# google-research/frame-interpolation

Hardware: NVIDIA H100
Metric: interpolated_frames_per_sec_1080p (higher is better)
Workload: dtype f16x2-split (activations/weights as fp16 hi+lo planes; fp32 accumulate)

## Files before the change

frame_interpolation_b200/csrc/film_conv.h:

```cpp
#pragma once
#include <cuda.h>
#include <stdint.h>

#include "film_common.cuh"

namespace film {

constexpr int kMaxSrc = 4;
constexpr int kMaxTaps = 9;
constexpr int kChunk = 64;
constexpr int kTileM = 128;

struct ConvSrc {
  const sp_t* hi;
  const sp_t* lo;
  int C;
  int c_off;
  int nchunk;
  int bswap;
};

struct alignas(64) ConvProblem {
  CUtensorMap tm_a_hi[kMaxSrc];
  CUtensorMap tm_a_lo[kMaxSrc];
  CUtensorMap tm_w_hi;
  CUtensorMap tm_w_lo;
  CUtensorMap tm_w_hi_half;
  CUtensorMap tm_w_lo_half;
  ConvSrc src[kMaxSrc];
  int nsrc;
  int B, H, W;
  int tile_h, tile_w;
  int tiles_y, tiles_x;
  int ntaps;
  int tap_dy[kMaxTaps], tap_dx[kMaxTaps];
  int kchunk;
  int ktot;
  const sp_t* w_hi;
  const sp_t* w_lo;
  const float* bias;
  int cout;
  int act;
  sp_t* out_hi;
  sp_t* out_lo;
  int out_C, out_c_off;
  int out_H, out_W;
  int out_sy, out_sx, out_oy, out_ox;
  int epi_mode;
  const float* head_w3;
  const float* head_b3;
  int crop_y, crop_x, crop_h, crop_w;
  int64_t crop_pitch;
  const float* head_w4;
  const float* head_b4;
  const float* head_vup;
  float* head_res;
  float* head_v;
  int v2_resident;
  int v2_na, v2_nw;
  int v2_grid;
  int v2_part_lo, v2_part_hi;
  sp_t* pool_hi;
  sp_t* pool_lo;
  int pool_C;
  int group;
  int pair;
  int halo;
  int bn;
  int passes;
  int straight;
  int out_lo_skip;
};

cudaError_t launch_conv_tc(const ConvProblem* d_prob, const ConvProblem& h_prob, cudaStream_t st);
cudaError_t launch_conv_simt(const ConvProblem* d_prob, const ConvProblem& h_prob, cudaStream_t st);
cudaError_t conv_tc_configure();
bool conv3x3_tc_plan(ConvProblem& h_prob, int num_sms);
void conv3x3_tc_pick_tile(int H, int W, int B, int cout, int kc, int passes, int ktot, int epi_mode, int num_sms,
                          int& tile_h, int& tile_w);
cudaError_t launch_conv3x3_tc(const ConvProblem* d_prob, const ConvProblem& h_prob, cudaStream_t st);
cudaError_t conv3x3_tc_configure();
}
```

frame_interpolation_b200/csrc/film_conv3x3_tc.cu:

```cuda
#include <cuda.h>
#include <cuda_runtime.h>
#include <stdint.h>

#include <type_traits>

#include "film_conv.h"
#include "film_tc_ptx.cuh"

namespace film {
namespace {
using namespace tc;

constexpr int kConsumers = 256;
constexpr int kThreads = kConsumers + 128;
__host__ __device__ constexpr int a_plane_bytes(int kc, int th, int tw) { return (th + 2) * tw * kc * 2; }
__host__ __device__ constexpr int a_stage_bytes(int kc, int th, int tw) { return 2 * a_plane_bytes(kc, th, tw); }
constexpr int kHaloW = 10, kHaloRows = 18;
__host__ __device__ constexpr int halo_box_bytes(int kc) { return kHaloRows * kHaloW * kc * 2; }
__host__ __device__ constexpr int halo_plane_bytes(int kc) { return (halo_box_bytes(kc) + 1023) & ~1023; }
__host__ __device__ constexpr int a_stage_bytes_h(int kc, int th, int tw, int halo, int planes = 2) {
  return planes * (halo ? halo_plane_bytes(kc) : a_plane_bytes(kc, th, tw));
}
constexpr int kMaxRing = 8;
constexpr int kSmemLimit = 227 * 1024;
constexpr int kBarBytes = 8 * (4 * kMaxRing + 4);
constexpr int kFixedBytes = kBarBytes + 16 + 512 * 4  + 64  + 1024  + 64;
constexpr int kHeadW3 = 64 * 32 * 4, kHeadMisc = 512;
constexpr int kHeadBytes = kHeadW3 + kHeadMisc;

__host__ __device__ inline int w_tap_bytes(int bn, int kc, int planes = 2) { return bn * kc * 2 * planes; }

template <int BN, int KC, bool kPartial, bool kHalo, bool kOne, bool kRes>
__global__ void __launch_bounds__(kThreads, 1) k_conv3x3_tc(const ConvProblem* __restrict__ prob) {
  extern __shared__ uint8_t smem_raw[];
  constexpr bool one = kOne;
  const int planes = one ? 1 : 2;
  constexpr int kWPlane = BN * KC * 2;
  const int kWTap = kWPlane * planes;
  const int kTileH = prob->tile_h, kTileW = prob->tile_w;
  constexpr int kHaloBox = halo_box_bytes(KC), kHaloPlane = halo_plane_bytes(KC);
  constexpr bool halo = kHalo;
  const int kAPlane = halo ? kHaloPlane : a_plane_bytes(KC, kTileH, kTileW);
  const int kAStage = planes * kAPlane;
  const int kRowStep = kTileW * KC * 2;
  constexpr bool kFused = BN <= 128;
  constexpr int kAccRegs = (kFused ? 2 * BN : BN) / 2;

  const int NA = prob->v2_na, NW = prob->v2_nw;
  const bool resident = prob->v2_resident != 0;
  const int nsrc = prob->nsrc;
  const int tiles_x = prob->tiles_x, tiles_per_img = prob->tiles_y * prob->tiles_x;
  const int cout = prob->cout;
  const int n_nt = (cout + BN - 1) / BN;
  const int ntiles = prob->B * tiles_per_img * n_nt;
  int nkb = 0;
  for (int s = 0; s < nsrc; ++s) nkb += prob->src[s].nchunk * 9;

  const FastDiv div_nt(n_nt, ntiles), div_img(tiles_per_img, ntiles), div_tx(tiles_x, ntiles);
  const bool pair = prob->pair != 0;
  const int rank = pair ? (int)cluster_ctarank() : 0;
  const int nsp = prob->B * tiles_per_img;
  const int nwork = pair ? ((nsp + 1) / 2) * n_nt : ntiles;
  const int w_first = pair ? (int)blockIdx.x >> 1 : (int)blockIdx.x, w_step = pair ? (int)gridDim.x >> 1 : (int)gridDim.x;
  auto decode = [&](int work, int& sp, int& nti) {
    div_nt.divmod(work, sp, nti);
    if (pair) sp = 2 * sp + rank;
  };

  const uint32_t raw = smem_u32(smem_raw);
  const uint32_t base = (raw + 1023u) & ~1023u;
  uint8_t* gen_base = smem_raw + (base - raw);
  const uint32_t a_base = base;
  const uint32_t w_base = a_base + (uint32_t)NA * kAStage;
  const uint32_t w_bytes = resident ? (uint32_t)nkb * kWTap : (uint32_t)NW * kWTap;
  const uint32_t tail = w_base + w_bytes;
  const uint32_t tail_off = (uint32_t)NA * kAStage + w_bytes;
  float* bias_smem = reinterpret_cast<float*>(gen_base + tail_off + kBarBytes + 16);
  int* src_tab = reinterpret_cast<int*>(gen_base + tail_off + kBarBytes + 16 + 512 * 4);

  const int warp = threadIdx.x >> 5, lane = threadIdx.x & 31;

  if (warp == 8 && lane == 0) {
    for (int s = 0; s < kMaxRing; ++s) {
      mbar_init(tail + 8u * s, 1);
      mbar_init(tail + 8u * (kMaxRing + s), 2);
      mbar_init(tail + 8u * (2 * kMaxRing + s), 1);
      mbar_init(tail + 8u * (3 * kMaxRing + s), pair ? 4 : 2);
    }
    for (int s = 0; s < kMaxSrc; ++s) {
      src_tab[2 * s] = s < nsrc ? prob->src[s].nchunk : 0;
      src_tab[2 * s + 1] = s < nsrc ? prob->src[s].c_off : 0;
      src_tab[2 * kMaxSrc + s] = s < nsrc ? prob->src[s].bswap : 0;
    }
    asm volatile("fence.mbarrier_init.release.cluster;" ::: "memory");
  }
  if (warp < 8)
    for (int i = threadIdx.x; i < n_nt * BN; i += kConsumers) bias_smem[i] = (i < cout) ? prob->bias[i] : 0.f;
  __syncthreads();
  if (pair) cluster_sync_all();
  auto leave = [&]() {
    if (pair) cluster_sync_all();
  };

  if (warp >= 8) {
    regs_dec<40>();
    if (warp > 8) {
      leave();
      return;
    }
    const CUtensorMap* tm_w_hi = &prob->tm_w_hi;
    const CUtensorMap* tm_w_lo = &prob->tm_w_lo;
    if (resident && elect_one()) {
      mbar_expect_tx(tail + 8u * (2 * kMaxRing), (uint32_t)nkb * kWTap);
      for (int kb = 0; kb < nkb; ++kb) {
        tma_load_2d(w_base + kb * kWTap, tm_w_hi, tail + 8u * (2 * kMaxRing), kb * KC, 0);
        if (!one) tma_load_2d(w_base + kb * kWTap + kWPlane, tm_w_lo, tail + 8u * (2 * kMaxRing), kb * KC, 0);
      }
    }
    __syncwarp();
    RingPos ra, rw;
    for (int tile = w_first; tile < nwork; tile += w_step) {
      int sp, nti, b, rem, ty, tx;
      decode(tile, sp, nti);
      div_img.divmod(sp, b, rem);
      div_tx.divmod(rem, ty, tx);
      const int n0 = nti * BN, y0 = ty * kTileH, x0 = tx * kTileW;
      {
        const int nt = tile + w_step;
        int next_sp, nnt;
        decode(nt < nwork ? nt : 0, next_sp, nnt);
        if (nt < nwork && next_sp != sp && next_sp < nsp && elect_one()) {
          int nb, nrem, nty, ntx;
          div_img.divmod(next_sp, nb, nrem);
          div_tx.divmod(nrem, nty, ntx);
          const int ny0 = nty * kTileH, nx0 = ntx * kTileW;
          for (int s = 0; s < nsrc; ++s)
            for (int ch = 0; ch < src_tab[2 * s]; ++ch) {
              const int cc = src_tab[2 * s + 1] + ch * KC;
              tma_prefetch_4d(&prob->tm_a_hi[s], cc, nx0 - 1, ny0 - 1, nb);
              if (!one) tma_prefetch_4d(&prob->tm_a_lo[s], cc, nx0 - 1, ny0 - 1, nb);
              if (!halo) {
                tma_prefetch_4d(&prob->tm_a_hi[s], cc, nx0 + 1, ny0 - 1, nb);
                if (!one) tma_prefetch_4d(&prob->tm_a_lo[s], cc, nx0 + 1, ny0 - 1, nb);
              }
            }
        }
        __syncwarp();
      }
      int kb = 0;
      for (int s = 0; s < nsrc; ++s) {
        const int nchunk = src_tab[2 * s], c_off = src_tab[2 * s + 1];
        const int bs = src_tab[2 * kMaxSrc + s] ? prob->B - 1 - b : b;
        const CUtensorMap* tm_hi = &prob->tm_a_hi[s];
        const CUtensorMap* tm_lo = &prob->tm_a_lo[s];
        for (int ch = 0; ch < nchunk; ++ch) {
          const int nst = halo ? 1 : 3;
          for (int dx = 0; dx < nst; ++dx) {
            const int st = ra.stage;
            mbar_wait(tail + 8u * (kMaxRing + st), ra.phase ^ 1u);
            if (elect_one()) {
              const uint32_t sa = a_base + st * kAStage, bar = tail + 8u * st;
              mbar_expect_tx(bar, halo ? (uint32_t)(planes * kHaloBox) : (uint32_t)kAStage);
              tma_load_4d(sa, tm_hi, bar, c_off + ch * KC, x0 + dx - 1, y0 - 1, bs);
              if (!one) tma_load_4d(sa + kAPlane, tm_lo, bar, c_off + ch * KC, x0 + dx - 1, y0 - 1, bs);
            }
            __syncwarp();
            ra.advance(NA);
            if (!resident) {
              const int ntap = halo ? 9 : 3;
              for (int t = 0; t < ntap; ++t, ++kb) {
                const int ws = rw.stage;
                mbar_wait(tail + 8u * (3 * kMaxRing + ws), rw.phase ^ 1u);
                if (elect_one()) {
                  const uint32_t sw = w_base + ws * kWTap, bar = tail + 8u * (2 * kMaxRing + ws);
                  mbar_expect_tx(bar, kWTap);
                  if (pair) {
                    const uint32_t hoff = (uint32_t)(rank * (kWPlane / 2));
                    tma_load_2d_mc(sw + hoff, &prob->tm_w_hi_half, bar, kb * KC, n0 + rank * (BN / 2), 3);
                    if (!one) tma_load_2d_mc(sw + kWPlane + hoff, &prob->tm_w_lo_half, bar, kb * KC, n0 + rank * (BN / 2), 3);
                  } else {
                    tma_load_2d(sw, tm_w_hi, bar, kb * KC, n0);
                    if (!one) tma_load_2d(sw + kWPlane, tm_w_lo, bar, kb * KC, n0);
                  }
                }
                __syncwarp();
                rw.advance(NW);
              }
            }
          }
        }
      }
    }
    leave();
    return;
  }

  regs_inc<232>();
  const int wg = warp >> 2;
  const int q = lane & 3;
  const int H = prob->H, W = prob->W, out_H = prob->out_H, out_W = prob->out_W, out_C = prob->out_C;
  const int out_c_off = prob->out_c_off, act = prob->act;
  sp_t* const out_hi = prob->out_hi;
  sp_t* const out_lo = prob->out_lo;
  sp_t* const pool_hi = prob->pool_hi;
  sp_t* const pool_lo = prob->pool_lo;
  const int pool_C = prob->pool_C;
  const bool do_pool = pool_hi != nullptr;
  const bool lo_skip = prob->out_lo_skip != 0;
  const bool rgb = prob->epi_mode == 2;
  const float* const head_w = prob->head_w4;
  float* const rgb_out = prob->head_v;
  const int crop_y = prob->crop_y, crop_x = prob->crop_x, crop_h = prob->crop_h, crop_w = prob->crop_w;
  const int64_t crop_pitch = prob->crop_pitch;
  const bool fhead = prob->epi_mode == 3;
  constexpr int kHid = BN <= 64 ? BN / 2 : 1;
  float* const w3s = reinterpret_cast<float*>(reinterpret_cast<uint8_t*>(src_tab) + 64);
  float* const hmisc = w3s + kHeadW3 / 4;
  if (fhead) {
    if constexpr (BN <= 64) {
      for (int i = threadIdx.x; i < BN * kHid; i += kConsumers) w3s[i] = prob->head_w3[i];
      for (int i = threadIdx.x; i < kHid; i += kConsumers) hmisc[i] = prob->head_b3[i];
      for (int i = threadIdx.x; i < 2 * kHid; i += kConsumers) hmisc[kHid + i] = prob->head_w4[i];
      if (threadIdx.x < 2) hmisc[3 * kHid + threadIdx.x] = prob->head_b4[threadIdx.x];
    }
    asm volatile("bar.sync 1, %0;" ::"r"(kConsumers) : "memory");
  }
  const float* const head_vup = prob->head_vup;
  float* const head_res = prob->head_res;
  float* const head_vout = prob->head_v;

  if (resident) mbar_wait(tail + 8u * (2 * kMaxRing), 0);
  const bool is_leader = (threadIdx.x & 127) == 0;
  const uint32_t w_empty_peer = pair ? map_to_cta(tail + 8u * (3 * kMaxRing), (uint32_t)(rank ^ 1)) : 0u;
  auto release_w = [&](int slot) {
    mbar_arrive(tail + 8u * (3 * kMaxRing + slot));
    if (pair) mbar_arrive_cluster(w_empty_peer + 8u * slot);
  };
  {
    constexpr int kWTapC = kWPlane * (kOne ? 1 : 2);
    constexpr int kStageTaps = kHalo ? 9 : 3;
    constexpr uint32_t kPx = KC * 2;
    const int nab = nkb / kStageTaps;
    [[maybe_unused]] const int part_lo = prob->v2_part_lo, part_hi = prob->v2_part_hi;
    const uint32_t a_row0 = kHalo ? (uint32_t)(wg * 8 * kHaloW) * kPx : (uint32_t)(wg * 64) * kPx;
    const uint32_t sbo = kHalo ? kHaloW * kPx : 8 * kPx;
    RingPos ra, rw;
    float acc[kAccRegs];
    for (int tile = w_first; tile < nwork; tile += w_step) {
      int kb = 0;
      int rel_a = -1, rel_w = -1;
      auto retire = [&](int next_a, int next_w) {
        wgmma_commit();
        wgmma_wait<1>();
        if (is_leader) {
          if (rel_a >= 0) mbar_arrive(tail + 8u * (kMaxRing + rel_a));
          if (rel_w >= 0) release_w(rel_w);
        }
        rel_a = next_a;
        rel_w = next_w;
      };
      auto stage = [&](auto ksteps_c) {
        constexpr int kSteps = decltype(ksteps_c)::value;
        const int st = ra.stage;
        mbar_wait(tail + 8u * st, ra.phase);
        const uint32_t sa = a_base + st * kAStage + a_row0;
        const uint32_t lo_off = (uint32_t)(kHalo ? kHaloPlane : kAPlane);
        if constexpr (kRes) {
          const uint64_t a0 = make_desc_sbo<KC>(sa, sbo);
          const uint64_t lo_delta = (uint64_t)(lo_off >> 4);
          const uint64_t row_delta = (uint64_t)(kRowStep >> 4);
          const uint64_t w0 = make_desc_kc<KC>(w_base + kb * kWTapC);
          const uint32_t first = (kb == 0) ? 0u : 1u;
          wgmma_fence();
#pragma unroll
          for (int t = 0; t < kStageTaps; ++t) {
            const uint64_t a_hi = a0 + (kHalo ? (uint64_t)((((t % 3) * kHaloW + t / 3) * kPx) >> 4) : (uint64_t)t * row_delta);
            const uint64_t a_lo = a_hi + lo_delta;
            const uint64_t w_hi = w0 + (uint64_t)((t * kWTapC) >> 4), w_lo = w_hi + (uint64_t)(kWPlane >> 4);
#pragma unroll
            for (int k = 0; k < kSteps; ++k) {
              const uint64_t adv = (uint64_t)(k * 32 >> 4);
              const uint32_t accf = (t == 0 && k == 0) ? first : 1u;
              if constexpr (kOne) {
                wgmma<BN>(acc, a_hi + adv, w_hi + adv, accf);
              } else if constexpr (kFused) {
                wgmma<BN>(acc, a_hi + adv, w_hi + adv, accf);
                wgmma<BN>(acc + BN / 2, a_hi + adv, w_lo + adv, accf);
                wgmma<BN>(acc, a_lo + adv, w_hi + adv, 1u);
              } else {
                wgmma<BN>(acc, a_lo + adv, w_hi + adv, accf);
                wgmma<BN>(acc, a_hi + adv, w_lo + adv, 1u);
                wgmma<BN>(acc, a_hi + adv, w_hi + adv, 1u);
              }
            }
          }
          retire(st, -1);
          kb += kStageTaps;
        } else {
          for (int t = 0; t < kStageTaps; ++t, ++kb) {
            uint32_t sw;
            int ws = -1;
            if (resident) {
              sw = w_base + kb * kWTap;
            } else {
              ws = rw.stage;
              mbar_wait(tail + 8u * (2 * kMaxRing + ws), rw.phase);
              sw = w_base + ws * kWTap;
            }
            const uint32_t off = kHalo ? (uint32_t)((t % 3) * kHaloW + t / 3) * kPx : (uint32_t)(t * kRowStep);
            const uint64_t a_hi = make_desc_sbo<KC>(sa + off, sbo);
            const uint64_t a_lo = make_desc_sbo<KC>(sa + lo_off + off, sbo);
            const uint64_t w_hi = make_desc_kc<KC>(sw), w_lo = make_desc_kc<KC>(sw + kWPlane);
            const uint32_t first = (kb == 0) ? 0u : 1u;
            wgmma_fence();
#pragma unroll
            for (int k = 0; k < kSteps; ++k) {
              const uint64_t adv = (uint64_t)(k * 32 >> 4);
              if constexpr (kOne) {
                wgmma<BN>(acc, a_hi + adv, w_hi + adv, k == 0 ? first : 1u);
              } else if constexpr (kFused) {
                wgmma<BN>(acc, a_hi + adv, w_hi + adv, k == 0 ? first : 1u);
                wgmma<BN>(acc + BN / 2, a_hi + adv, w_lo + adv, k == 0 ? first : 1u);
                wgmma<BN>(acc, a_lo + adv, w_hi + adv, 1u);
              } else {
                wgmma<BN>(acc, a_lo + adv, w_hi + adv, k == 0 ? first : 1u);
                wgmma<BN>(acc, a_hi + adv, w_lo + adv, 1u);
                wgmma<BN>(acc, a_hi + adv, w_hi + adv, 1u);
              }
            }
            retire(t == kStageTaps - 1 ? st : -1, ws);
            if (!resident) rw.advance(NW);
          }
        }
        ra.advance(NA);
      };
      using Full = std::integral_constant<int, KC / 16>;
      if constexpr (kPartial) {
        for (int ab = 0; ab < part_lo; ++ab) stage(Full{});
        for (int ab = part_lo; ab < part_hi; ++ab) stage(std::integral_constant<int, 1>{});
        for (int ab = part_hi; ab < nab; ++ab) stage(Full{});
      } else {
        for (int ab = 0; ab < nab; ++ab) stage(Full{});
      }
      wgmma_wait<0>();
      if (is_leader) {
        if (rel_a >= 0) mbar_arrive(tail + 8u * (kMaxRing + rel_a));
        if (rel_w >= 0) release_w(rel_w);
      }
      acc_fence<kAccRegs>(acc);

      int sp, nti, b, rem, ty, tx;
      decode(tile, sp, nti);
      div_img.divmod(sp, b, rem);
      div_tx.divmod(rem, ty, tx);
      const int n0 = nti * BN;
      const bool live = sp < nsp;
      auto value = [&](int h, int j, int e) {
        const int i = 4 * j + 2 * h + e;
        return (kFused && !kOne) ? acc[i] + acc[(i + BN / 2) % kAccRegs] : acc[i];
      };
#pragma unroll
      for (int h = 0; h < 2 && (fhead || rgb); ++h) {
        const int r = wg * 64 + (warp & 3) * 16 + (lane >> 2) + 8 * h;
        const int py = ty * kTileH + r / kTileW, px = tx * kTileW + r % kTileW;
        const bool valid = live && (py < H) && (px < W);
        const int64_t opix = ((int64_t)b * out_H + py) * out_W + px;
        if (fhead) {
          if constexpr (BN <= 64) {
            float hp[kHid];
#pragma unroll
            for (int hh = 0; hh < kHid; ++hh) hp[hh] = 0.f;
#pragma unroll
            for (int j = 0; j < BN / 8; ++j)
#pragma unroll
              for (int e = 0; e < 2; ++e) {
                const int c = 8 * j + 2 * q + e;
                const float x = value(h, j, e) + bias_smem[n0 + c];
                const float f = act ? leaky(x) : x;
                const float4* wr = reinterpret_cast<const float4*>(w3s + c * kHid);
#pragma unroll
                for (int h4 = 0; h4 < kHid / 4; ++h4) {
                  const float4 wv = wr[h4];
                  hp[4 * h4] = fmaf(f, wv.x, hp[4 * h4]);
                  hp[4 * h4 + 1] = fmaf(f, wv.y, hp[4 * h4 + 1]);
                  hp[4 * h4 + 2] = fmaf(f, wv.z, hp[4 * h4 + 2]);
                  hp[4 * h4 + 3] = fmaf(f, wv.w, hp[4 * h4 + 3]);
                }
              }
#pragma unroll
            for (int hh = 0; hh < kHid; ++hh) {
              hp[hh] += __shfl_xor_sync(0xffffffffu, hp[hh], 1);
              hp[hh] += __shfl_xor_sync(0xffffffffu, hp[hh], 2);
            }
            if (q == 0 && valid) {
              float f0 = hmisc[3 * kHid], f1 = hmisc[3 * kHid + 1];
#pragma unroll
              for (int hh = 0; hh < kHid; ++hh) {
                const float x = leaky(hp[hh] + hmisc[hh]);
                f0 = fmaf(x, hmisc[kHid + 2 * hh], f0);
                f1 = fmaf(x, hmisc[kHid + 2 * hh + 1], f1);
              }
              float2 res = make_float2(f0, f1), tot = res;
              if (head_vup) {
                const float2 u = reinterpret_cast<const float2*>(head_vup)[opix];
                tot.x += u.x;
                tot.y += u.y;
              }
              reinterpret_cast<float2*>(head_res)[opix] = res;
              reinterpret_cast<float2*>(head_vout)[opix] = tot;
            }
          }
        } else if (rgb) {
          float r0 = 0.f, r1 = 0.f, r2 = 0.f;
#pragma unroll
          for (int j = 0; j < BN / 8; ++j)
#pragma unroll
            for (int e = 0; e < 2; ++e) {
              const int c = n0 + 8 * j + 2 * q + e;
              float f = value(h, j, e) + bias_smem[c];
              if (act) f = leaky(f);
              r0 = fmaf(f, __ldg(head_w + 3 * c), r0);
              r1 = fmaf(f, __ldg(head_w + 3 * c + 1), r1);
              r2 = fmaf(f, __ldg(head_w + 3 * c + 2), r2);
            }
#pragma unroll
          for (int m = 1; m <= 2; m <<= 1) {
            r0 += __shfl_xor_sync(0xffffffffu, r0, m);
            r1 += __shfl_xor_sync(0xffffffffu, r1, m);
            r2 += __shfl_xor_sync(0xffffffffu, r2, m);
          }
          const int oy = py - crop_y, ox = px - crop_x;
          if (q == 0 && valid && oy >= 0 && oy < crop_h && ox >= 0 && ox < crop_w) {
            float* o = rgb_out + (int64_t)oy * crop_pitch + (int64_t)ox * 3;
            o[0] = r0 + __ldg(prob->head_b4);
            o[1] = r1 + __ldg(prob->head_b4 + 1);
            o[2] = r2 + __ldg(prob->head_b4 + 2);
          }
        }
      }
      if (!fhead && !rgb) {
        bool valid[2];
        int64_t opix[2];
#pragma unroll
        for (int h = 0; h < 2; ++h) {
          const int r = wg * 64 + (warp & 3) * 16 + (lane >> 2) + 8 * h;
          const int py = ty * kTileH + r / kTileW, px = tx * kTileW + r % kTileW;
          valid[h] = live && (py < H) && (px < W);
          opix[h] = ((int64_t)b * out_H + py) * out_W + px;
        }
        const int r0 = wg * 64 + (warp & 3) * 16 + (lane >> 2);
        const int64_t ppix = ((int64_t)b * (out_H >> 1) + ((ty * kTileH + r0 / kTileW) >> 1)) * (out_W >> 1) +
                             ((tx * kTileW + r0 % kTileW) >> 1);
#pragma unroll
        for (int j = 0; j < BN / 8; ++j) {
          const int c = 8 * j + 2 * q;
          if (n0 + c >= cout) break;
          float a[2][2];
#pragma unroll
          for (int h = 0; h < 2; ++h) {
            float f0 = value(h, j, 0) + bias_smem[n0 + c], f1 = value(h, j, 1) + bias_smem[n0 + c + 1];
            if (act) {
              f0 = leaky(f0);
              f1 = leaky(f1);
            }
            if (valid[h]) {
              sp_t* oh = out_hi + opix[h] * out_C + out_c_off + n0;
              if (lo_skip) {
                *reinterpret_cast<uint32_t*>(oh + c) = pack2_hi(f0, f1);
              } else {
                sp_t* ol = out_lo + opix[h] * out_C + out_c_off + n0;
                uint32_t hi, lo;
                split_pack2(f0, f1, hi, lo);
                *reinterpret_cast<uint32_t*>(oh + c) = hi;
                *reinterpret_cast<uint32_t*>(ol + c) = lo;
              }
            }
            if (do_pool) {
              a[h][0] = f0 + __shfl_xor_sync(0xffffffffu, f0, 4);
              a[h][1] = f1 + __shfl_xor_sync(0xffffffffu, f1, 4);
            }
          }
          if (do_pool && valid[0] && !(lane & 4)) {
            uint32_t hi, lo;
            split_pack2((a[0][0] + a[1][0]) * 0.25f, (a[0][1] + a[1][1]) * 0.25f, hi, lo);
            *reinterpret_cast<uint32_t*>(pool_hi + ppix * pool_C + n0 + c) = hi;
            *reinterpret_cast<uint32_t*>(pool_lo + ppix * pool_C + n0 + c) = lo;
          }
        }
      }
    }
  }
  leave();
}

int smem_bytes_for(const ConvProblem& h, int bn) {
  const int nkb = h.ktot / h.kchunk;
  const int planes = h.passes == 1 ? 1 : 2;
  const int w = h.v2_resident ? nkb * w_tap_bytes(bn, h.kchunk, planes) : h.v2_nw * w_tap_bytes(bn, h.kchunk, planes);
  return h.v2_na * a_stage_bytes_h(h.kchunk, h.tile_h, h.tile_w, h.halo, planes) + w + kFixedBytes +
         (h.epi_mode == 3 ? kHeadBytes : 0);
}

}

int conv_tc_block_n(int cout);

namespace {
bool ring_depths(int kc, int tile_h, int tile_w, int halo, int planes, int bn, int cout, int ktot, int epi_mode,
                 int& resident, int& na, int& nw) {
  const int wtap = w_tap_bytes(bn, kc, planes);
  const int w_all = (ktot / kc) * wtap;
  const int kLimit = kSmemLimit - (epi_mode == 3 ? kHeadBytes : 0);
  const int kAStage = a_stage_bytes_h(kc, tile_h, tile_w, halo, planes);
  if (cout <= bn && w_all + 2 * kAStage + kFixedBytes <= kLimit) {
    resident = 1;
    const int n = (kLimit - kFixedBytes - w_all) / kAStage;
    const int n_max = halo ? 3 : 6;
    na = n > n_max ? n_max : n;
    nw = 1;
    return true;
  }
  resident = 0;
  na = halo ? 2 : (bn >= 128 ? 2 : 3);
  int n = (kLimit - kFixedBytes - na * kAStage) / wtap;
  if (n < 2 && na > 2) {
    na = 2;
    n = (kLimit - kFixedBytes - na * kAStage) / wtap;
  }
  nw = n > kMaxRing ? kMaxRing : n;
  return nw >= 2;
}
}

void conv3x3_tc_pick_tile(int H, int W, int B, int cout, int kc, int passes, int ktot, int epi_mode, int num_sms,
                          int& tile_h, int& tile_w) {
  static const int cand[3][2] = {{16, 8}, {8, 16}, {4, 32}};
  const int bn = conv_tc_block_n(cout);
  const int n_nt = (cout + bn - 1) / bn;
  double best = 1e30;
  tile_h = 16;
  tile_w = 8;
  for (auto& c : cand) {
    int res, na, nw;
    if (!ring_depths(kc, c[0], c[1], 0, passes == 1 ? 1 : 2, bn, cout, ktot, epi_mode, res, na, nw)) continue;
    const long tiles = (long)B * ((H + c[0] - 1) / c[0]) * ((W + c[1] - 1) / c[1]) * n_nt;
    const long waves = (tiles + num_sms - 1) / num_sms;
    const double cost = (double)waves * (c[0] + 2.0) / c[0] * (1.0 + 1e-3 * (c[1] / 8));
    if (cost < best) {
      best = cost;
      tile_h = c[0];
      tile_w = c[1];
    }
  }
}

bool conv3x3_tc_plan(ConvProblem& h, int num_sms) {
  const int bn = h.bn;
  const int planes = h.passes == 1 ? 1 : 2;
  const int wtap = w_tap_bytes(bn, h.kchunk, planes);
  const int w_all = (h.ktot / h.kchunk) * wtap;
  const bool can_resident = h.cout <= bn;
  const int kLimit = kSmemLimit - (h.epi_mode == 3 ? kHeadBytes : 0);
  if (h.halo && (h.tile_h != 16 || h.tile_w != 8 ||
                 (can_resident && w_all + 2 * a_stage_bytes_h(h.kchunk, h.tile_h, h.tile_w, 0, planes) + kFixedBytes <= kLimit &&
                  w_all + 2 * a_stage_bytes_h(h.kchunk, h.tile_h, h.tile_w, 1, planes) + kFixedBytes > kLimit)))
    h.halo = 0;
  bool ok = ring_depths(h.kchunk, h.tile_h, h.tile_w, h.halo, planes, bn, h.cout, h.ktot, h.epi_mode, h.v2_resident,
                        h.v2_na, h.v2_nw);
  if (!ok && h.halo) {
    h.halo = 0;
    ok = ring_depths(h.kchunk, h.tile_h, h.tile_w, 0, planes, bn, h.cout, h.ktot, h.epi_mode, h.v2_resident, h.v2_na,
                     h.v2_nw);
  }
  const int nsp = h.B * h.tiles_y * h.tiles_x, n_nt = (h.cout + bn - 1) / bn;
  if (h.pair) {
    const int nwork = (nsp + 1) / 2 * n_nt, nclu = num_sms / 2;
    h.v2_grid = 2 * (nwork < nclu ? nwork : nclu);
  } else {
    h.v2_grid = nsp * n_nt < num_sms ? nsp * n_nt : num_sms;
  }
  return ok;
}

template <int BN, int KC>
struct Variants {
  static constexpr void (*kFn[16])(const ConvProblem*) = {
      k_conv3x3_tc<BN, KC, false, false, false, false>, k_conv3x3_tc<BN, KC, false, false, false, true>,
      k_conv3x3_tc<BN, KC, false, false, true, false>,  k_conv3x3_tc<BN, KC, false, false, true, true>,
      k_conv3x3_tc<BN, KC, false, true, false, false>,  k_conv3x3_tc<BN, KC, false, true, false, true>,
      k_conv3x3_tc<BN, KC, false, true, true, false>,   k_conv3x3_tc<BN, KC, false, true, true, true>,
      k_conv3x3_tc<BN, KC, true, false, false, false>,  k_conv3x3_tc<BN, KC, true, false, false, true>,
      k_conv3x3_tc<BN, KC, true, false, true, false>,   k_conv3x3_tc<BN, KC, true, false, true, true>,
      k_conv3x3_tc<BN, KC, true, true, false, false>,   k_conv3x3_tc<BN, KC, true, true, false, true>,
      k_conv3x3_tc<BN, KC, true, true, true, false>,    k_conv3x3_tc<BN, KC, true, true, true, true>};
  static cudaError_t configure() {
    for (auto fn : kFn) {
      const cudaError_t e = cudaFuncSetAttribute(fn, cudaFuncAttributeMaxDynamicSharedMemorySize, kSmemLimit);
      if (e != cudaSuccess) return e;
    }
    return cudaSuccess;
  }
  static cudaError_t launch(const ConvProblem* d_prob, const ConvProblem& h, cudaStream_t st) {
    if (h.v2_na < 2 || (!h.v2_resident && h.v2_nw < 2)) return cudaErrorInvalidValue;
    const bool partial = h.v2_part_hi > h.v2_part_lo;
    const int idx = (partial ? 8 : 0) | (h.halo ? 4 : 0) | (h.passes == 1 ? 2 : 0) | (h.v2_resident && h.straight ? 1 : 0);
    if (!h.pair) {
      kFn[idx]<<<h.v2_grid, kThreads, smem_bytes_for(h, BN), st>>>(d_prob);
      return cudaGetLastError();
    }
    cudaLaunchConfig_t cfg = {};
    cudaLaunchAttribute attr[1];
    attr[0].id = cudaLaunchAttributeClusterDimension;
    attr[0].val.clusterDim.x = 2;
    attr[0].val.clusterDim.y = 1;
    attr[0].val.clusterDim.z = 1;
    cfg.gridDim = dim3(h.v2_grid);
    cfg.blockDim = dim3(kThreads);
    cfg.dynamicSmemBytes = smem_bytes_for(h, BN);
    cfg.stream = st;
    cfg.attrs = attr;
    cfg.numAttrs = 1;
    return cudaLaunchKernelEx(&cfg, kFn[idx], d_prob);
  }
};

cudaError_t conv3x3_tc_configure() {
  cudaError_t e;
#define FILM_CFG(BN, KC)                        \
  e = Variants<BN, KC>::configure();            \
  if (e != cudaSuccess) return e;
  FILM_CFG(32, 64) FILM_CFG(64, 64) FILM_CFG(128, 64) FILM_CFG(256, 64) FILM_CFG(32, 32) FILM_CFG(64, 32)
#undef FILM_CFG
  return cudaSuccess;
}

cudaError_t launch_conv3x3_tc(const ConvProblem* d_prob, const ConvProblem& h, cudaStream_t st) {
  const int bn = h.bn;
  if (h.kchunk == 32) {
    if (bn == 32) return Variants<32, 32>::launch(d_prob, h, st);
    if (bn == 64) return Variants<64, 32>::launch(d_prob, h, st);
    return cudaErrorInvalidValue;
  }
  switch (bn) {
    case 256: return Variants<256, 64>::launch(d_prob, h, st);
    case 128: return Variants<128, 64>::launch(d_prob, h, st);
    case 64: return Variants<64, 64>::launch(d_prob, h, st);
    default: return Variants<32, 64>::launch(d_prob, h, st);
  }
}

}
```

frame_interpolation_b200/csrc/film_engine.cu:

```cuda
#include <cuda.h>
#include <cuda_runtime.h>

#include <algorithm>
#include <cmath>
#include <cstdio>
#include <cstdlib>
#include <cstring>
#include <functional>
#include <map>
#include <memory>
#include <string>
#include <vector>

#include "../../include/film_b200.h"
#include "film_conv.h"
#include "film_kernels.h"

namespace film {
int conv_tc_block_n(int cout);

constexpr int kLevels = 7, kFusionLevels = 5, kSpecialized = 3, kSubLevels = 4, kFilters = 64;
static const int kFlowFilters[4] = {32, 64, 128, 256};
static const char* kPredictorNames[4] = {"flow_predictor_0", "flow_predictor_1", "flow_predictor_2",
                                         "flow_predictor_shared"};
static int feat_channels(int l) {
  int c = 0;
  for (int j = 0; j <= (l < kSubLevels - 1 ? l : kSubLevels - 1); ++j) c += kFilters << j;
  return c;
}
static int fusion_filters(int l) { return l < kSpecialized ? (kFilters << l) : (kFilters << kSpecialized); }
static int round_up(int a, int b) { return (a + b - 1) / b * b; }

struct Error {
  int code;
  std::string msg;
};

enum Stage {
  ST_FE_I0_K01 = 0, ST_FE_I0_K23, ST_FE_I0_K45, ST_FE_I0_K67,
  ST_FE_I1, ST_FE_I2, ST_FE_I3P,
  ST_FLOW_L0,
  ST_FUS = ST_FLOW_L0 + kLevels,
  ST_COUNT = ST_FUS + 3 * (kFusionLevels - 1),
  ST_NONE = -1
};
static std::string stage_name(int s) {
  static const char* fe[] = {"fe_i0_k01", "fe_i0_k23", "fe_i0_k45", "fe_i0_k67", "fe_i1", "fe_i2", "fe_i3p"};
  if (s < 0 || s >= ST_COUNT) return "";
  if (s < ST_FLOW_L0) return fe[s];
  if (s < ST_FUS) return "flow_L" + std::to_string(s - ST_FLOW_L0);
  return "fus" + std::to_string((s - ST_FUS) / 3) + "_c" + std::to_string((s - ST_FUS) % 3);
}
static int fe_stage(int image_level, int conv_k) {
  if (image_level == 0) return ST_FE_I0_K01 + conv_k / 2;
  return image_level == 1 ? ST_FE_I1 : image_level == 2 ? ST_FE_I2 : ST_FE_I3P;
}
constexpr uint32_t kDefaultOnepassMask =
    (1u << ST_FE_I0_K23) | (1u << ST_FE_I0_K45) | (1u << ST_FE_I0_K67) |
    (0x1Fu << ST_FLOW_L0) | (0x3Fu << (ST_FUS + 6));
#define FILM_CUDA(expr)                                                                       \
  do {                                                                                        \
    cudaError_t e__ = (expr);                                                                 \
    if (e__ != cudaSuccess)                                                                   \
      throw Error{FILM_ERR_CUDA, std::string(#expr) + ": " + cudaGetErrorString(e__)};        \
  } while (0)

struct HostTensor {
  std::vector<int> dims;
  std::vector<float> data;
};
typedef std::map<std::string, HostTensor> WeightMap;

static WeightMap read_weight_file(const char* path) {
  FILE* f = fopen(path, "rb");
  if (!f) throw Error{FILM_ERR_WEIGHTS, std::string("cannot open weight file ") + path};
  WeightMap m;
  auto fail = [&](const char* why) {
    fclose(f);
    throw Error{FILM_ERR_WEIGHTS, std::string(path) + ": " + why};
  };
  char magic[8];
  if (fread(magic, 1, 8, f) != 8 || memcmp(magic, "FILMW1\0\0", 8) != 0) fail("bad magic");
  uint32_t n;
  if (fread(&n, 4, 1, f) != 1) fail("truncated");
  for (uint32_t i = 0; i < n; ++i) {
    uint32_t ln, nd;
    if (fread(&ln, 4, 1, f) != 1 || ln > 4096) fail("bad name length");
    std::string name(ln, '\0');
    if (fread(&name[0], 1, ln, f) != ln) fail("truncated");
    if (fread(&nd, 4, 1, f) != 1 || nd > 8) fail("bad rank");
    HostTensor t;
    size_t cnt = 1;
    for (uint32_t d = 0; d < nd; ++d) {
      uint32_t v;
      if (fread(&v, 4, 1, f) != 1) fail("truncated");
      t.dims.push_back((int)v);
      cnt *= v;
    }
    t.data.resize(cnt);
    if (fread(t.data.data(), 4, cnt, f) != cnt) fail("truncated tensor data");
    m[name] = std::move(t);
  }
  fclose(f);
  return m;
}

static const HostTensor& get_tensor(const WeightMap& m, const std::string& name, std::vector<int> dims) {
  auto it = m.find(name);
  if (it == m.end()) throw Error{FILM_ERR_WEIGHTS, "missing tensor " + name};
  if (it->second.dims != dims) throw Error{FILM_ERR_WEIGHTS, "shape mismatch for " + name};
  return it->second;
}

static uint16_t f32_to_bf16(float f) {
  uint32_t u;
  memcpy(&u, &f, 4);
  if ((u & 0x7fffffffu) > 0x7f800000u) return (uint16_t)((u >> 16) | 0x40);
  u += 0x7fffu + ((u >> 16) & 1u);
  return (uint16_t)(u >> 16);
}
static float bf16_to_f32(uint16_t h) {
  uint32_t u = (uint32_t)h << 16;
  float f;
  memcpy(&f, &u, 4);
  return f;
}
static uint16_t f32_to_sp(float f) {
#ifdef FILM_SPLIT_FP16
  __half h = __float2half_rn(f);
  uint16_t u;
  memcpy(&u, &h, 2);
  return u;
#else
  return f32_to_bf16(f);
#endif
}
static float sp_to_f32(uint16_t h) {
#ifdef FILM_SPLIT_FP16
  __half v;
  memcpy(&v, &h, 2);
  return __half2float(v);
#else
  return bf16_to_f32(h);
#endif
}

struct PackedConv {
  sp_t* w_hi = nullptr;
  sp_t* w_lo = nullptr;
  float* bias = nullptr;
  int cout = 0, ktot = 0, cin_ref = 0;
  int kchunk = kChunk;
  std::vector<int> src_chunks;
  std::vector<int> src_ksteps;
  int ntaps = 0;
  int tap_dy[kMaxTaps], tap_dx[kMaxTaps];
};

struct TapSpec {
  int dy, dx;
  std::vector<std::pair<int, int>> terms;
};

static PackedConv pack_conv(const HostTensor& kernel, const HostTensor& bias,
                            const std::vector<std::vector<int>>& src_maps,
                            const std::vector<TapSpec>& taps, std::vector<void*>& allocs, int chunk = kChunk) {
  const int kw = kernel.dims[1], cin = kernel.dims[2], cout = kernel.dims[3];
  PackedConv pc;
  pc.cout = cout;
  pc.cin_ref = cin;
  pc.kchunk = chunk;
  pc.ntaps = (int)taps.size();
  for (size_t t = 0; t < taps.size(); ++t) {
    pc.tap_dy[t] = taps[t].dy;
    pc.tap_dx[t] = taps[t].dx;
  }
  int ktot = 0;
  for (auto& sm : src_maps) {
    if (sm.size() % chunk) throw Error{FILM_ERR_WEIGHTS, "source channel map not a multiple of the K chunk"};
    pc.src_chunks.push_back((int)sm.size() / chunk);
    int ks = 1;
    for (size_t i = 0; i < sm.size(); ++i)
      if (sm[i] >= 0) ks = std::max(ks, (int)(i % chunk) / 16 + 1);
    pc.src_ksteps.push_back(ks);
    ktot += (int)sm.size() * (int)taps.size();
  }
  pc.ktot = ktot;
  std::vector<uint16_t> hi((size_t)cout * ktot), lo((size_t)cout * ktot);
  int kbase = 0;
  for (auto& sm : src_maps) {
    const int nchunk = (int)sm.size() / chunk;
    for (int ch = 0; ch < nchunk; ++ch) {
      for (size_t t = 0; t < taps.size(); ++t, kbase += chunk) {
        for (int c = 0; c < chunk; ++c) {
          const int ref = sm[ch * chunk + c];
          for (int n = 0; n < cout; ++n) {
            float w = 0.f;
            if (ref >= 0) {
              if (ref >= cin) throw Error{FILM_ERR_WEIGHTS, "channel map out of range"};
              for (auto& term : taps[t].terms)
                w += kernel.data[(((size_t)term.first * kw + term.second) * cin + ref) * cout + n];
            }
            const uint16_t h = f32_to_sp(w);
            const uint16_t l = f32_to_sp(w - sp_to_f32(h));
            hi[(size_t)n * ktot + kbase + c] = h;
            lo[(size_t)n * ktot + kbase + c] = l;
          }
        }
      }
    }
  }
  FILM_CUDA(cudaMalloc(&pc.w_hi, hi.size() * 2));
  allocs.push_back(pc.w_hi);
  FILM_CUDA(cudaMalloc(&pc.w_lo, lo.size() * 2));
  allocs.push_back(pc.w_lo);
  FILM_CUDA(cudaMalloc(&pc.bias, cout * 4));
  allocs.push_back(pc.bias);
  FILM_CUDA(cudaMemcpy(pc.w_hi, hi.data(), hi.size() * 2, cudaMemcpyHostToDevice));
  FILM_CUDA(cudaMemcpy(pc.w_lo, lo.data(), lo.size() * 2, cudaMemcpyHostToDevice));
  FILM_CUDA(cudaMemcpy(pc.bias, bias.data.data(), cout * 4, cudaMemcpyHostToDevice));
  return pc;
}

static std::vector<TapSpec> taps_3x3() {
  std::vector<TapSpec> t;
  for (int kx = 0; kx < 3; ++kx)
    for (int ky = 0; ky < 3; ++ky) t.push_back({ky - 1, kx - 1, {{ky, kx}}});
  return t;
}
static std::vector<TapSpec> taps_up2x2(int py, int px) {
  std::vector<TapSpec> t;
  for (int dy = 0; dy <= py; ++dy)
    for (int dx = 0; dx <= px; ++dx) {
      TapSpec s{dy, dx, {}};
      for (int fy = 0; fy < 2; ++fy)
        for (int fx = 0; fx < 2; ++fx)
          if ((py + fy) / 2 == dy && (px + fx) / 2 == dx) s.terms.push_back({fy, fx});
      t.push_back(s);
    }
  return t;
}
static std::vector<int> iota_map(int start, int n, int padded) {
  std::vector<int> m(padded, -1);
  for (int i = 0; i < n; ++i) m[i] = start + i;
  return m;
}
static std::vector<int> side_map(int C) {
  std::vector<int> m(kChunk, -1);
  for (int c = 0; c < 3; ++c) m[c] = c;
  for (int c = 0; c < 3; ++c) m[3 + c] = 3 + C + c;
  m[6] = 6 + 2 * C;
  m[7] = 7 + 2 * C;
  m[8] = 8 + 2 * C;
  m[9] = 9 + 2 * C;
  return m;
}

struct Model {
  std::vector<void*> allocs;
  float *conv0_w = nullptr, *conv0_b = nullptr;
  PackedConv fe[8];
  PackedConv fe0_3x3;
  PackedConv flow[4][3];
  PackedConv flow_c3[4];
  float *flow_w3[4], *flow_b3[4], *flow_w4[4], *flow_b4[4];
  PackedConv fus_up[4][4];
  PackedConv fus_c1[4], fus_c2[4];
  float *rgb_w = nullptr, *rgb_b = nullptr;

  float* upload(const HostTensor& t) {
    float* d;
    FILM_CUDA(cudaMalloc(&d, t.data.size() * 4));
    allocs.push_back(d);
    FILM_CUDA(cudaMemcpy(d, t.data.data(), t.data.size() * 4, cudaMemcpyHostToDevice));
    return d;
  }

  void load(const WeightMap& w) {
    const std::string fe_pre = "feat_net/sub_extractor/cfeat_conv_";
    conv0_w = upload(get_tensor(w, fe_pre + "0/kernel", {3, 3, 3, 64}));
    conv0_b = upload(get_tensor(w, fe_pre + "0/bias", {64}));
    {
      HostTensor k0 = get_tensor(w, fe_pre + "0/kernel", {3, 3, 3, 64});
      k0.dims = {1, 1, 27, 64};
      fe[0] = pack_conv(k0, get_tensor(w, fe_pre + "0/bias", {64}), {iota_map(0, 27, 32)},
                        {TapSpec{0, 0, {{0, 0}}}}, allocs, 32);
      fe0_3x3 = pack_conv(get_tensor(w, fe_pre + "0/kernel", {3, 3, 3, 64}), get_tensor(w, fe_pre + "0/bias", {64}),
                          {iota_map(0, 3, 32)}, taps_3x3(), allocs, 32);
    }
    int cin = 64;
    for (int k = 1; k < 8; ++k) {
      const int c = kFilters << (k / 2);
      fe[k] = pack_conv(get_tensor(w, fe_pre + std::to_string(k) + "/kernel", {3, 3, cin, c}),
                        get_tensor(w, fe_pre + std::to_string(k) + "/bias", {c}),
                        {iota_map(0, cin, cin)}, taps_3x3(), allocs);
      cin = c;
    }
    for (int p = 0; p < 4; ++p) {
      const std::string pre = std::string("predict_flow/") + kPredictorNames[p] + "/conv_";
      const int nf = kFlowFilters[p], C = feat_channels(p);
      flow[p][0] = pack_conv(get_tensor(w, pre + "0/kernel", {3, 3, 2 * C, nf}),
                             get_tensor(w, pre + "0/bias", {nf}),
                             {iota_map(0, C, C), iota_map(C, C, C)}, taps_3x3(), allocs);
      const int kc = nf < kChunk ? 32 : kChunk;
      for (int k = 1; k < 3; ++k)
        flow[p][k] = pack_conv(get_tensor(w, pre + std::to_string(k) + "/kernel", {3, 3, nf, nf}),
                               get_tensor(w, pre + std::to_string(k) + "/bias", {nf}),
                               {iota_map(0, nf, round_up(nf, kc))}, taps_3x3(), allocs, kc);
      flow_c3[p] = pack_conv(get_tensor(w, pre + "3/kernel", {1, 1, nf, nf / 2}),
                             get_tensor(w, pre + "3/bias", {nf / 2}), {iota_map(0, nf, round_up(nf, kc))},
                             {TapSpec{0, 0, {{0, 0}}}}, allocs, kc);
      flow_w3[p] = upload(get_tensor(w, pre + "3/kernel", {1, 1, nf, nf / 2}));
      flow_b3[p] = upload(get_tensor(w, pre + "3/bias", {nf / 2}));
      flow_w4[p] = upload(get_tensor(w, pre + "4/kernel", {1, 1, nf / 2, 2}));
      flow_b4[p] = upload(get_tensor(w, pre + "4/bias", {2}));
    }
    for (int i = 0; i < kFusionLevels - 1; ++i) {
      const std::string pre = "fusion/level_" + std::to_string(i) + "/conv_";
      const int nf = fusion_filters(i), C = feat_channels(i);
      const bool from_pyr = (i == kFusionLevels - 2);
      const int Cc = feat_channels(i + 1);
      const int coarse_c = from_pyr ? 2 * (3 + Cc) + 4 : fusion_filters(i + 1);
      const HostTensor& k0 = get_tensor(w, pre + "0/kernel", {2, 2, coarse_c, nf});
      const HostTensor& b0 = get_tensor(w, pre + "0/bias", {nf});
      std::vector<std::vector<int>> up_src;
      if (from_pyr)
        up_src = {iota_map(3, Cc, Cc), iota_map(6 + Cc, Cc, Cc), side_map(Cc)};
      else
        up_src = {iota_map(0, coarse_c, coarse_c)};
      for (int py = 0; py < 2; ++py)
        for (int px = 0; px < 2; ++px)
          fus_up[i][py * 2 + px] = pack_conv(k0, b0, up_src, taps_up2x2(py, px), allocs);
      const int a_c = 2 * (3 + C) + 4;
      fus_c1[i] = pack_conv(get_tensor(w, pre + "1/kernel", {3, 3, a_c + nf, nf}),
                            get_tensor(w, pre + "1/bias", {nf}),
                            {iota_map(3, C, C), iota_map(6 + C, C, C), side_map(C),
                             iota_map(a_c, nf, round_up(nf, kChunk))},
                            taps_3x3(), allocs);
      fus_c2[i] = pack_conv(get_tensor(w, pre + "2/kernel", {3, 3, nf, nf}),
                            get_tensor(w, pre + "2/bias", {nf}),
                            {iota_map(0, nf, round_up(nf, kChunk))}, taps_3x3(), allocs);
    }
    rgb_w = upload(get_tensor(w, "fusion/output_conv/kernel", {1, 1, 64, 3}));
    rgb_b = upload(get_tensor(w, "fusion/output_conv/bias", {3}));
  }
  ~Model() {
    for (void* p : allocs) cudaFree(p);
  }
};

typedef CUresult (*EncodeTiledFn)(CUtensorMap*, CUtensorMapDataType, cuuint32_t, void*, const cuuint64_t*,
                                  const cuuint64_t*, const cuuint32_t*, const cuuint32_t*,
                                  CUtensorMapInterleave, CUtensorMapSwizzle, CUtensorMapL2promotion,
                                  CUtensorMapFloatOOBfill);
static EncodeTiledFn get_encode_fn() {
  static EncodeTiledFn fn = nullptr;
  if (!fn) {
    void* p = nullptr;
    cudaDriverEntryPointQueryResult qres;
    FILM_CUDA(cudaGetDriverEntryPoint("cuTensorMapEncodeTiled", &p, cudaEnableDefault, &qres));
    if (qres != cudaDriverEntryPointSuccess || !p)
      throw Error{FILM_ERR_CUDA, "cuTensorMapEncodeTiled entry point not available"};
    fn = (EncodeTiledFn)p;
  }
  return fn;
}
#ifdef FILM_SPLIT_FP16
static const CUtensorMapDataType kTmType = CU_TENSOR_MAP_DATA_TYPE_FLOAT16;
#else
static const CUtensorMapDataType kTmType = CU_TENSOR_MAP_DATA_TYPE_BFLOAT16;
#endif

static void make_act_map(CUtensorMap* tm, const sp_t* base, int B, int H, int W, int C, int th, int tw, int kc) {
  cuuint64_t dims[4] = {(cuuint64_t)C, (cuuint64_t)W, (cuuint64_t)H, (cuuint64_t)B};
  cuuint64_t strides[3] = {(cuuint64_t)C * 2, (cuuint64_t)W * C * 2, (cuuint64_t)H * W * C * 2};
  cuuint32_t box[4] = {(cuuint32_t)kc, (cuuint32_t)tw, (cuuint32_t)th, 1};
  cuuint32_t estr[4] = {1, 1, 1, 1};
  CUresult r = get_encode_fn()(tm, kTmType, 4, (void*)base, dims, strides, box, estr,
                               CU_TENSOR_MAP_INTERLEAVE_NONE, kc == 32 ? CU_TENSOR_MAP_SWIZZLE_64B : CU_TENSOR_MAP_SWIZZLE_128B,
                               CU_TENSOR_MAP_L2_PROMOTION_L2_256B, CU_TENSOR_MAP_FLOAT_OOB_FILL_NONE);
  if (r != CUDA_SUCCESS) throw Error{FILM_ERR_CUDA, "cuTensorMapEncodeTiled(activation) failed: " + std::to_string((int)r)};
}
static void make_w_map(CUtensorMap* tm, const sp_t* base, int cout, int ktot, int bn, int kc) {
  cuuint64_t dims[2] = {(cuuint64_t)ktot, (cuuint64_t)cout};
  cuuint64_t strides[1] = {(cuuint64_t)ktot * 2};
  cuuint32_t box[2] = {(cuuint32_t)kc, (cuuint32_t)bn};
  cuuint32_t estr[2] = {1, 1};
  CUresult r = get_encode_fn()(tm, kTmType, 2, (void*)base, dims, strides, box, estr,
                               CU_TENSOR_MAP_INTERLEAVE_NONE, kc == 32 ? CU_TENSOR_MAP_SWIZZLE_64B : CU_TENSOR_MAP_SWIZZLE_128B,
                               CU_TENSOR_MAP_L2_PROMOTION_L2_256B, CU_TENSOR_MAP_FLOAT_OOB_FILL_NONE);
  if (r != CUDA_SUCCESS) throw Error{FILM_ERR_CUDA, "cuTensorMapEncodeTiled(weights) failed: " + std::to_string((int)r)};
}

struct SplitBuf {
  sp_t* hi = nullptr;
  sp_t* lo = nullptr;
  int B = 0, H = 0, W = 0, C = 0;
  int64_t pixels() const { return (int64_t)B * H * W; }
};
struct SrcRef {
  const SplitBuf* buf;
  int c_off;
  int bswap;
};
struct DebugTensor {
  bool split;
  const void* p0;
  const void* p1;
  int64_t npix;
  int C, c_off, Cn;
  bool recycled = false;
};

struct Plan {
  int h, w, H, W, off_y, off_x;
  int conv_impl;
  int conv3x3_v2 = 1, num_sms = 132, conv3x3_2cta = 0;
  int conv3x3_halo = 0;
  uint32_t onepass_mask = 0;
  int fe_conv0_tc = 0;
  int fuse_rgb_head = 1;
  int fuse_flow_head = 1;
  int plane_skip = 1;
  int mma_straight = 1;
  std::vector<void*> allocs;
  int64_t arena_bytes = 0;
  std::vector<ConvProblem> h_probs;
  ConvProblem* d_probs = nullptr;
  struct Op {
    std::function<cudaError_t(cudaStream_t)> fn;
    int category;
    std::string name;
    double flops;
    double bytes;
    int lane;
    std::vector<int> waits;
    std::vector<int> signals;
  };
  std::vector<Op> ops;
  std::vector<float> op_ms;
  static constexpr int kNumLanes = 8;
  int cur_lane = 0, num_tokens = 0, tok_end = -1;
  std::vector<int> pending_waits;
  int new_token() { return num_tokens++; }
  void add_op(int category, const std::string& name, std::function<cudaError_t(cudaStream_t)> fn,
              double flops = 0, double bytes = 0) {
    ops.push_back(Op{std::move(fn), category, name, flops, bytes, cur_lane, pending_waits, {}});
    pending_waits.clear();
  }
  void signal_last(int token) { ops.back().signals.push_back(token); }
  std::map<std::string, DebugTensor> debug;
  float* xin = nullptr;
  float* xout = nullptr;
  cudaGraphExec_t graph = nullptr;
  double conv_flops = 0, mma_flops = 0, warp_bytes = 0, last_conv_bytes = 0;

  bool reuse = true;
  std::map<void*, int64_t> block_bytes;
  std::multimap<int64_t, void*> free_blocks;
  template <class T>
  T* alloc(int64_t count, bool pinned = false) {
    const int64_t bytes = std::max<int64_t>(count * (int64_t)sizeof(T), 256);
    if (reuse && !pinned) {
      auto it = free_blocks.lower_bound(bytes);
      if (it != free_blocks.end() && it->first <= 2 * bytes) {
        void* p = it->second;
        free_blocks.erase(it);
        return (T*)p;
      }
    }
    void* p;
    FILM_CUDA(cudaMalloc(&p, bytes));
    allocs.push_back(p);
    FILM_CUDA(cudaMemset(p, 0, bytes));
    arena_bytes += bytes;
    if (!pinned) block_bytes[p] = bytes;
    return (T*)p;
  }
  void release(void* p) {
    if (!reuse || !p) return;
    auto it = block_bytes.find(p);
    if (it != block_bytes.end()) free_blocks.insert({it->second, p});
  }
  void release(const SplitBuf* s) {
    if (!s) return;
    release((void*)s->hi);
    release((void*)s->lo);
  }
  SplitBuf* split(int B, int H_, int W_, int C, bool pinned = false) {
    bufs.emplace_back(new SplitBuf);
    SplitBuf* s = bufs.back().get();
    s->B = B;
    s->H = H_;
    s->W = W_;
    s->C = C;
    s->hi = alloc<sp_t>((int64_t)B * H_ * W_ * C, pinned);
    s->lo = alloc<sp_t>((int64_t)B * H_ * W_ * C, pinned);
    return s;
  }
  std::vector<std::unique_ptr<SplitBuf>> bufs;

  ~Plan() {
    if (graph) cudaGraphExecDestroy(graph);
    for (void* p : allocs) cudaFree(p);
  }
};

static void pick_tile(int H, int W, int& th, int& tw) {
  static const int cand[][2] = {{8, 16}, {16, 8}, {4, 32}, {32, 4}, {2, 64}, {64, 2}, {1, 128}, {128, 1}};
  long best = -1;
  for (auto& c : cand) {
    long tiles = (long)((H + c[0] - 1) / c[0]) * ((W + c[1] - 1) / c[1]);
    if (best < 0 || tiles < best) {
      best = tiles;
      th = c[0];
      tw = c[1];
    }
  }
}

static size_t add_conv(Plan& P, const std::string& tag, double ref_macs_per_px, const PackedConv& pc,
                       const std::vector<SrcRef>& sources, int act, const SplitBuf* out, int out_c_off,
                       int stage, int consumer, int sy = 1, int sx = 1, int oy = 0, int ox = 0,
                       const SplitBuf* pool_out = nullptr, bool no_op = false, int epi_mode = 0) {
  ConvProblem cp;
  memset(&cp, 0, sizeof(cp));
  cp.passes = (stage >= 0 && P.conv_impl == 0 && ((P.onepass_mask >> stage) & 1u)) ? 1 : 3;
  cp.out_lo_skip = (consumer >= 0 && P.conv_impl == 0 && !pool_out && P.plane_skip && ((P.onepass_mask >> consumer) & 1u)) ? 1 : 0;
  cp.straight = P.mma_straight;
  const SplitBuf* s0 = sources[0].buf;
  cp.nsrc = (int)sources.size();
  if (cp.nsrc != (int)pc.src_chunks.size()) throw Error{FILM_ERR_WEIGHTS, "source count mismatch"};
  cp.B = s0->B;
  cp.H = s0->H;
  cp.W = s0->W;
  const int kc = pc.kchunk;
  cp.kchunk = kc;
  const bool v2 = P.conv3x3_v2 && P.conv_impl == 0 && pc.ntaps == 9 && (out || epi_mode >= 2) && sy == 1 && sx == 1 &&
                  (kc == kChunk || pc.cout <= 64);
  cp.epi_mode = epi_mode;
  int box_h, box_w;
  if (v2) {
    if (pool_out) {
      cp.tile_h = 16;
      cp.tile_w = 8;
    } else {
      conv3x3_tc_pick_tile(cp.H, cp.W, cp.B, pc.cout, kc, cp.passes, pc.ktot, epi_mode, P.num_sms, cp.tile_h, cp.tile_w);
    }
    box_h = cp.tile_h + 2;
    box_w = cp.tile_w;
  } else {
    pick_tile(cp.H, cp.W, cp.tile_h, cp.tile_w);
    box_h = cp.tile_h;
    box_w = cp.tile_w;
  }
  cp.tiles_y = (cp.H + cp.tile_h - 1) / cp.tile_h;
  cp.tiles_x = (cp.W + cp.tile_w - 1) / cp.tile_w;
  for (int s = 0; s < cp.nsrc; ++s) {
    const SplitBuf* b = sources[s].buf;
    if (b->B != cp.B || b->H != cp.H || b->W != cp.W) throw Error{FILM_ERR_ARG, "conv source grid mismatch"};
    cp.src[s].hi = b->hi;
    cp.src[s].lo = b->lo;
    cp.src[s].C = b->C;
    cp.src[s].c_off = sources[s].c_off;
    cp.src[s].nchunk = pc.src_chunks[s];
    cp.src[s].bswap = sources[s].bswap;
    if (sources[s].c_off + pc.src_chunks[s] * kc > b->C) throw Error{FILM_ERR_ARG, "conv source channel overrun"};
    make_act_map(&cp.tm_a_hi[s], b->hi, b->B, b->H, b->W, b->C, box_h, box_w, kc);
    make_act_map(&cp.tm_a_lo[s], b->lo, b->B, b->H, b->W, b->C, box_h, box_w, kc);
  }
  cp.ntaps = pc.ntaps;
  for (int t = 0; t < pc.ntaps; ++t) {
    cp.tap_dy[t] = pc.tap_dy[t];
    cp.tap_dx[t] = pc.tap_dx[t];
  }
  cp.ktot = pc.ktot;
  cp.w_hi = pc.w_hi;
  cp.w_lo = pc.w_lo;
  cp.bias = pc.bias;
  cp.cout = pc.cout;
  cp.act = act;
  int bn = conv_tc_block_n(pc.cout);
  if (out && !pool_out) {
    auto items = [&](int b) { return (long)cp.B * cp.tiles_y * cp.tiles_x * ((pc.cout + b - 1) / b); };
    while (bn > 64 && 2 * items(bn) <= P.num_sms) bn /= 2;
  }
  cp.bn = bn;
  make_w_map(&cp.tm_w_hi, pc.w_hi, pc.cout, pc.ktot, bn, kc);
  make_w_map(&cp.tm_w_lo, pc.w_lo, pc.cout, pc.ktot, bn, kc);
  make_w_map(&cp.tm_w_hi_half, pc.w_hi, pc.cout, pc.ktot, bn / 2, kc);
  make_w_map(&cp.tm_w_lo_half, pc.w_lo, pc.cout, pc.ktot, bn / 2, kc);
  if (out) {
    cp.out_hi = out->hi;
    cp.out_lo = out->lo;
    cp.out_C = out->C;
    cp.out_H = out->H;
    cp.out_W = out->W;
  } else {
    cp.out_C = 0;
    cp.out_H = cp.H;
    cp.out_W = cp.W;
  }
  cp.out_c_off = out_c_off;
  cp.out_sy = sy;
  cp.out_sx = sx;
  cp.out_oy = oy;
  cp.out_ox = ox;
  if (out && (out->B != cp.B || out_c_off + pc.cout > out->C)) throw Error{FILM_ERR_ARG, "conv destination mismatch"};
  if (pool_out) {
    if (!v2) throw Error{FILM_ERR_UNSUPPORTED, "fused pool needs the persistent 3x3 kernel"};
    cp.pool_hi = pool_out->hi;
    cp.pool_lo = pool_out->lo;
    cp.pool_C = pool_out->C;
  }
  cp.group = 1;
  int halo_ok = (v2 && cp.tile_h == 16 && cp.tile_w == 8) ? P.conv3x3_halo : 0;
  if (kc != kChunk && halo_ok < 3) halo_ok = 0;
  cp.halo = halo_ok >= 2;
  if (v2 && !conv3x3_tc_plan(cp, P.num_sms))
    throw Error{FILM_ERR_UNSUPPORTED, "persistent 3x3 conv: shared-memory rings do not fit (" + tag + ")"};
  if (v2 && P.conv3x3_2cta && epi_mode < 2 && !cp.v2_resident &&
      (P.conv3x3_2cta >= 2 || (long)cp.B * cp.tiles_y * cp.tiles_x >= 4L * P.num_sms)) {
    cp.pair = 1;
    if (halo_ok >= 1) cp.halo = 1;
    if (!conv3x3_tc_plan(cp, P.num_sms))
      throw Error{FILM_ERR_UNSUPPORTED, "persistent 3x3 conv: shared-memory rings do not fit (" + tag + ")"};
  }
  if (cp.halo) {
    for (int s = 0; s < cp.nsrc; ++s) {
      const SplitBuf* b = sources[s].buf;
      make_act_map(&cp.tm_a_hi[s], b->hi, b->B, b->H, b->W, b->C, box_h, box_w + 2, kc);
      make_act_map(&cp.tm_a_lo[s], b->lo, b->B, b->H, b->W, b->C, box_h, box_w + 2, kc);
    }
  }
  if (v2) {
    const int nst = cp.halo ? 1 : 3;
    for (int s = 0, ab = 0; s < cp.nsrc; ab += pc.src_chunks[s] * nst, ++s) {
      if (pc.src_chunks[s] == 0 || pc.src_ksteps[s] == kc / 16) continue;
      if (pc.src_ksteps[s] != 1 || cp.v2_part_hi > cp.v2_part_lo)
        throw Error{FILM_ERR_UNSUPPORTED, "persistent 3x3 conv: only one source may skip k-steps, and it must issue one (" +
                                              tag + ")"};
      cp.v2_part_lo = ab;
      cp.v2_part_hi = ab + pc.src_chunks[s] * nst;
    }
  }
  const size_t idx = P.h_probs.size();
  P.h_probs.push_back(cp);
  double k_issued = 0;
  for (size_t si = 0; si < pc.src_chunks.size(); ++si)
    k_issued += (double)pc.src_chunks[si] * pc.ntaps * (v2 ? pc.src_ksteps[si] * 16 : pc.kchunk);
  P.mma_flops += (double)cp.passes * 2.0 * (double)cp.B * cp.tiles_y * cp.tiles_x * kTileM * k_issued *
                 (double)(((pc.cout + bn - 1) / bn) * bn);
  double alg_bytes = 0;
  {
    const double px = (double)cp.B * cp.H * cp.W, planes_in = cp.passes == 1 ? 1.0 : 2.0;
    for (size_t si = 0; si < pc.src_chunks.size(); ++si) alg_bytes += px * pc.src_chunks[si] * pc.kchunk * 2.0 * planes_in;
    if (out) alg_bytes += px * pc.cout * 2.0 * (cp.out_lo_skip ? 1.0 : 2.0);
    if (pool_out) alg_bytes += px / 4.0 * pc.cout * 4.0;
    if (epi_mode == 2) alg_bytes += px * 12.0;
    if (!out && epi_mode != 2) alg_bytes += px * 24.0;
    alg_bytes += (double)pc.cout * pc.ktot * 2.0 * planes_in;
  }
  P.last_conv_bytes = alg_bytes;
  if (no_op) return idx;
  Plan* pp = &P;
  const int impl = P.conv_impl;
  P.add_op(0, tag, [pp, idx, impl, v2](cudaStream_t st) {
    if (impl == 1) return launch_conv_simt(pp->d_probs + idx, pp->h_probs[idx], st);
    return v2 ? launch_conv3x3_tc(pp->d_probs + idx, pp->h_probs[idx], st)
              : launch_conv_tc(pp->d_probs + idx, pp->h_probs[idx], st);
  }, 2.0 * ref_macs_per_px * (double)cp.B * cp.H * cp.W, alg_bytes);
  return idx;
}

static std::unique_ptr<Plan> build_plan(const Model& M, int h, int w, int align, int conv_impl, bool keep_debug,
                                        int conv3x3_v2, int num_sms, int conv3x3_2cta, int conv3x3_halo,
                                        uint32_t onepass_mask, bool use_lanes, int fe_conv0_tc) {
  std::unique_ptr<Plan> pl(new Plan);
  Plan& P = *pl;
  P.fe_conv0_tc = fe_conv0_tc & 1;
  P.fuse_rgb_head = (fe_conv0_tc & 2) ? 0 : 1;
  P.plane_skip = (fe_conv0_tc & 8) ? 0 : 1;
  P.fuse_flow_head = (fe_conv0_tc & 64) ? 0 : ((fe_conv0_tc & 128) ? 2 : 1);
  P.mma_straight = (fe_conv0_tc & 16) ? 0 : 1;
  P.onepass_mask = onepass_mask;
  P.reuse = !keep_debug && !use_lanes && !(fe_conv0_tc & 32);
  P.h = h;
  P.w = w;
  P.conv_impl = conv_impl;
  P.conv3x3_v2 = conv3x3_v2;
  P.conv3x3_2cta = conv3x3_2cta;
  P.conv3x3_halo = conv3x3_halo;
  P.num_sms = num_sms;
  int ph = 0, pw = 0;
  if (align > 0) {
    ph = (h % align) ? align - h % align : 0;
    pw = (w % align) ? align - w % align : 0;
  }
  P.H = h + ph;
  P.W = w + pw;
  P.off_y = ph / 2;
  P.off_x = pw / 2;
  if (P.H % 64 || P.W % 64)
    throw Error{FILM_ERR_UNSUPPORTED,
                "padded frame size must be a multiple of 64 (2^(pyramid_levels-1)) in this engine; use align=64"};
  int Hs[kLevels], Ws[kLevels];
  for (int l = 0; l < kLevels; ++l) {
    Hs[l] = P.H >> l;
    Ws[l] = P.W >> l;
  }
  if (Hs[kLevels - 2] < 2 || Ws[kLevels - 2] < 2) throw Error{FILM_ERR_ARG, "frame too small"};

  P.xin = P.alloc<float>((int64_t)2 * h * w * 3, true);
  P.xout = P.alloc<float>((int64_t)h * w * 3, true);
  Plan* pp = &P;

  float* img[kLevels];
  for (int l = 0; l < kLevels; ++l) img[l] = P.alloc<float>((int64_t)2 * Hs[l] * Ws[l] * 3, true);
  for (int k = 0; k < 2; ++k) {
    float* dst = img[0] + (int64_t)k * P.H * P.W * 3;
    const float* src = P.xin + (int64_t)k * h * w * 3;
    P.add_op(2, "pad_image", [=](cudaStream_t st) {
      return launch_pad_image(src, (int64_t)pp->w * 3, pp->h, pp->w, dst, pp->H, pp->W, pp->off_y, pp->off_x, st);
    });
  }
  const bool fuse_img_pool = P.conv_impl == 0 && !P.fe_conv0_tc && !use_lanes;
  for (int l = 0; l + 1 < kLevels && !fuse_img_pool; ++l) {
    const float* in = img[l];
    float* out = img[l + 1];
    const int hh = Hs[l], ww = Ws[l];
    P.add_op(2, "image_pool@L" + std::to_string(l), [=](cudaStream_t st) { return launch_image_pool(in, out, 2, hh, ww, st); });
  }

  const int tok_img = P.new_token();
  P.signal_last(tok_img);

  SplitBuf* feat[kLevels];
  for (int l = 0; l < kLevels; ++l) feat[l] = P.split(2, Hs[l], Ws[l], feat_channels(l));
  static const int slice_off[4] = {0, 64, 192, 448};
  int tok_feat[kLevels][kSubLevels];
  for (int i = 0; i < kLevels; ++i) {
    const int depth = (kLevels - i) < kSubLevels ? (kLevels - i) : kSubLevels;
    SplitBuf* pooled = nullptr;
    P.cur_lane = i;
    if (i > 0) P.pending_waits = {tok_img};
    for (int j = 0; j < depth; ++j) {
      const int r = i + j, c = kFilters << j;
      SplitBuf* t1 = P.split(2, Hs[r], Ws[r], c);
      if (j == 0 && P.conv_impl == 0 && !P.fe_conv0_tc) {
        const float* im = img[i];
        const int hh = Hs[r], ww = Ws[r];
        const float *w0 = M.conv0_w, *b0 = M.conv0_b;
        sp_t *oh = t1->hi, *ol = t1->lo;
        const bool lo_skip = P.plane_skip && ((P.onepass_mask >> fe_stage(i, 1)) & 1u);
        float* pool_dst = (fuse_img_pool && i + 1 < kLevels) ? img[i + 1] : nullptr;
        P.add_op(2, std::string(pool_dst ? "fe_conv0+pool@L" : "fe_conv0@L") + std::to_string(r),
                 [=](cudaStream_t st) { return launch_fe_conv0(im, 2, hh, ww, w0, b0, oh, ol, lo_skip, pool_dst, st); },
                 2.0 * 27 * 64 * 2.0 * hh * ww, 2.0 * hh * ww * (3 * 4 + 64 * (lo_skip ? 2.0 : 4.0)));
      } else if (j == 0 && P.conv_impl == 0 && P.conv3x3_v2) {
        const float* im = img[i];
        const int hh = Hs[r], ww = Ws[r];
        SplitBuf* im32 = P.split(2, hh, ww, 32, true);
        P.add_op(2, "fe_split32@L" + std::to_string(r),
                 [=](cudaStream_t st) { return launch_image_to_split32(im, 2, hh, ww, im32->hi, im32->lo, st); }, 0,
                 2.0 * hh * ww * (12 + 32.0));
        add_conv(P, "fe_conv0@L" + std::to_string(r), 27.0 * 64, M.fe0_3x3, {{im32, 0}}, 1, t1, 0, fe_stage(i, 0), fe_stage(i, 1));
      } else if (j == 0 && P.conv_impl == 0) {
        const float* im = img[i];
        const int hh = Hs[r], ww = Ws[r];
        SplitBuf* col = P.split(2, hh, ww, 32, true);
        P.add_op(2, "fe_im2col@L" + std::to_string(r),
                 [=](cudaStream_t st) { return launch_im2col3x3(im, 2, hh, ww, col->hi, col->lo, st); }, 0,
                 2.0 * hh * ww * (12 + 128.0));
        add_conv(P, "fe_conv0@L" + std::to_string(r), 27.0 * 64, M.fe[0], {{col, 0}}, 1, t1, 0, fe_stage(i, 0), fe_stage(i, 1));
      } else if (j == 0) {
        const float* im = img[i];
        const int hh = Hs[r], ww = Ws[r];
        const float *w0 = M.conv0_w, *b0 = M.conv0_b;
        sp_t *oh = t1->hi, *ol = t1->lo;
        P.add_op(2, "fe_conv0@L" + std::to_string(r),
                 [=](cudaStream_t st) { return launch_conv0_c3(im, 2, hh, ww, w0, b0, oh, ol, 64, 0, st); },
                 2.0 * 27 * 64 * 2.0 * hh * ww, 2.0 * hh * ww * (3 + 64) * 4.0);
      } else {
        add_conv(P, "fe_conv" + std::to_string(2 * j) + "@L" + std::to_string(r), 9.0 * (c / 2) * c, M.fe[2 * j],
                 {{pooled, 0}}, 1, t1, 0, fe_stage(i, 2 * j), fe_stage(i, 2 * j + 1));
        P.release(pooled);
      }
      SplitBuf* pool_target = nullptr;
      const bool fuse_pool = (j < depth - 1) && P.conv_impl == 0 && P.conv3x3_v2;
      if (j < depth - 1) pool_target = P.split(2, Hs[r + 1], Ws[r + 1], c);
      add_conv(P, "fe_conv" + std::to_string(2 * j + 1) + "@L" + std::to_string(r), 9.0 * c * c, M.fe[2 * j + 1],
               {{t1, 0}}, 1, feat[r], slice_off[j], fe_stage(i, 2 * j + 1), ST_NONE, 1, 1, 0, 0,
               fuse_pool ? pool_target : nullptr);
      P.release(t1);
      tok_feat[i][j] = P.new_token();
      P.signal_last(tok_feat[i][j]);
      if (fuse_pool) {
        pooled = pool_target;
      } else if (j < depth - 1) {
        pooled = pool_target;
        const SplitBuf* f = feat[r];
        const SplitBuf* po = pooled;
        const int so = slice_off[j];
        P.add_op(2, "fe_pool@L" + std::to_string(r), [=](cudaStream_t st) {
          return launch_act_pool(f->hi, f->lo, f->C, so, 2, f->H, f->W, c, po->hi, po->lo, po->C, st);
        });
      }
    }
  }
  for (int l = 0; l < kLevels; ++l)
    for (int k = 0; k < 2; ++k)
      P.debug["feat" + std::to_string(k) + "/" + std::to_string(l)] =
          DebugTensor{true, feat[l]->hi + (int64_t)k * Hs[l] * Ws[l] * feat[l]->C,
                      feat[l]->lo + (int64_t)k * Hs[l] * Ws[l] * feat[l]->C, (int64_t)Hs[l] * Ws[l], feat[l]->C, 0,
                      feat[l]->C};

  float* v[kLevels];
  float* res[kLevels];
  for (int l = 0; l < kLevels; ++l) {
    v[l] = P.alloc<float>((int64_t)2 * Hs[l] * Ws[l] * 2, true);
    res[l] = P.alloc<float>((int64_t)2 * Hs[l] * Ws[l] * 2, true);
  }
  P.cur_lane = Plan::kNumLanes - 1;
  for (int l = kLevels - 1; l >= 0; --l) {
    const int p = l < kSpecialized ? l : kSpecialized;
    const int nf = kFlowFilters[p], C = feat_channels(l), hh = Hs[l], ww = Ws[l];
    for (int i = (l - (kSubLevels - 1) > 0 ? l - (kSubLevels - 1) : 0); i <= l; ++i) P.pending_waits.push_back(tok_feat[i][l - i]);
    const SplitBuf* second;
    float* vup = nullptr;
    if (l == kLevels - 1) {
      second = nullptr;
    } else {
      SplitBuf* warped = P.split(2, hh, ww, C);
      vup = P.alloc<float>((int64_t)2 * hh * ww * 2);
      const float* vprev = v[l + 1];
      const SplitBuf* f = feat[l];
      const int hc = Hs[l + 1], wc = Ws[l + 1];
      float* vu = vup;
      const bool hi_only = P.conv_impl == 0 && P.plane_skip && ((P.onepass_mask >> (ST_FLOW_L0 + l)) & 1u);
      const double wbytes = 2.0 * hh * ww * (double)C * (hi_only ? 4.0 : 8.0);
      P.add_op(1, "flow_warp@L" + std::to_string(l), [=](cudaStream_t st) {
        return launch_flow_warp(vprev, hc, wc, f->hi, f->lo, hh, ww, C, vu, warped->hi, warped->lo, hi_only, st);
      }, 0, wbytes);
      P.warp_bytes += wbytes;
      second = warped;
      for (int d = 0; d < 2; ++d) {
        P.debug["flow_warped" + std::to_string(d) + "/" + std::to_string(l)] =
            DebugTensor{true, warped->hi + (int64_t)d * hh * ww * C, warped->lo + (int64_t)d * hh * ww * C, (int64_t)hh * ww,
                        C, 0, C};
        P.debug["flow_vup" + std::to_string(d) + "/" + std::to_string(l)] =
            DebugTensor{false, vup + (int64_t)d * hh * ww * 2, nullptr, (int64_t)hh * ww, 2, 0, 2};
      }
    }
    const int cpad = round_up(nf, nf < kChunk ? 32 : kChunk);
    SplitBuf* c0 = P.split(2, hh, ww, cpad);
    SplitBuf* c1 = P.split(2, hh, ww, cpad);
    SplitBuf* c2 = P.split(2, hh, ww, cpad);
    const std::string lt = "@L" + std::to_string(l);
    std::vector<SrcRef> flow_src(2);
    flow_src[0].buf = feat[l];
    flow_src[0].c_off = 0;
    flow_src[1].buf = second ? second : feat[l];
    flow_src[1].c_off = 0;
    flow_src[1].bswap = second ? 0 : 1;
    add_conv(P, "flow_conv0" + lt, 9.0 * 2 * C * nf, M.flow[p][0], flow_src, 1, c0, 0, ST_FLOW_L0 + l, ST_FLOW_L0 + l);
    add_conv(P, "flow_conv1" + lt, 9.0 * nf * nf, M.flow[p][1], {{c0, 0}}, 1, c1, 0, ST_FLOW_L0 + l, ST_FLOW_L0 + l);
    const bool fuse_head = P.conv_impl == 0 && P.conv3x3_v2 && P.fuse_flow_head && nf <= (P.fuse_flow_head >= 2 ? 64 : 32);
    if (fuse_head) {
      const size_t ci = add_conv(P, "flow_conv2+head" + lt, 9.0 * nf * nf + 1.0 * nf * (nf / 2) + (nf / 2) * 2.0, M.flow[p][2],
                                 {{c1, 0}}, 1, nullptr, 0, ST_FLOW_L0 + l, ST_NONE, 1, 1, 0, 0, nullptr, false, 3);
      ConvProblem& hp = P.h_probs[ci];
      if (hp.bn != nf) throw Error{FILM_ERR_UNSUPPORTED, "flow-head epilogue expects one N tile on the single-CTA kernel"};
      hp.head_w3 = M.flow_w3[p];
      hp.head_b3 = M.flow_b3[p];
      hp.head_w4 = M.flow_w4[p];
      hp.head_b4 = M.flow_b4[p];
      hp.head_vup = vup;
      hp.head_res = res[l];
      hp.head_v = v[l];
    } else {
      add_conv(P, "flow_conv2" + lt, 9.0 * nf * nf, M.flow[p][2], {{c1, 0}}, 1, c2, 0, ST_FLOW_L0 + l, ST_NONE);
    }
    if (fuse_head) {
    } else if (P.conv_impl == 1) {
      const float *w3 = M.flow_w3[p], *b3 = M.flow_b3[p], *w4 = M.flow_w4[p], *b4 = M.flow_b4[p];
      float *rr = res[l], *vv = v[l];
      const float* vu = vup;
      const int npix = 2 * hh * ww;
      P.add_op(2, "flow_head" + lt, [=](cudaStream_t st) {
        return launch_flow_head(c2->hi, c2->lo, c2->C, nf, npix, w3, b3, w4, b4, vu, rr, vv, st);
      });
    } else {
      const size_t ci = add_conv(P, "flow_head" + lt, 1.0 * nf * (nf / 2) + (nf / 2) * 2.0, M.flow_c3[p], {{c2, 0}}, 1,
                                 nullptr, 0, ST_NONE, ST_NONE);
      ConvProblem& hp = P.h_probs[ci];
      hp.epi_mode = 1;
      hp.head_w4 = M.flow_w4[p];
      hp.head_b4 = M.flow_b4[p];
      hp.head_vup = vup;
      hp.head_res = res[l];
      hp.head_v = v[l];
    }
    P.release(second);
    P.release(vup);
    P.release(c0);
    P.release(c1);
    P.release(c2);
    if (l >= kFusionLevels) P.release(feat[l]);
    const int64_t np = (int64_t)hh * ww;
    P.debug["flow_fwd/" + std::to_string(l)] = DebugTensor{false, v[l], nullptr, np, 2, 0, 2};
    P.debug["flow_bwd/" + std::to_string(l)] = DebugTensor{false, v[l] + np * 2, nullptr, np, 2, 0, 2};
    P.debug["res_fwd/" + std::to_string(l)] = DebugTensor{false, res[l], nullptr, np, 2, 0, 2};
    P.debug["res_bwd/" + std::to_string(l)] = DebugTensor{false, res[l] + np * 2, nullptr, np, 2, 0, 2};
  }

  SplitBuf* wf[kFusionLevels];
  SplitBuf* side[kFusionLevels];
  for (int l = 0; l < kFusionLevels; ++l) {
    const int C = feat_channels(l), hh = Hs[l], ww = Ws[l];
    wf[l] = P.split(2, hh, ww, C);
    side[l] = P.split(1, hh, ww, kChunk, true);
    const float* vv = v[l];
    const float* im = img[l];
    const SplitBuf *f = feat[l], *o = wf[l], *sd = side[l];
    const int cons = l == kFusionLevels - 1 ? ST_FUS + 3 * (l - 1) : ST_FUS + 3 * l + 1;
    const bool hi_only = P.conv_impl == 0 && P.plane_skip && ((P.onepass_mask >> cons) & 1u);
    const double wbytes = 2.0 * hh * ww * (double)C * (hi_only ? 4.0 : 8.0);
    P.add_op(1, "fusion_warp@L" + std::to_string(l), [=](cudaStream_t st) {
      return launch_fusion_warp(vv, f->hi, f->lo, hh, ww, C, o->hi, o->lo, hi_only, st);
    }, 0, wbytes);
    P.add_op(2, "fusion_side@L" + std::to_string(l), [=](cudaStream_t st) {
      return launch_fusion_side(vv, im, hh, ww, sd->hi, sd->lo, sd->C, st);
    });
    P.warp_bytes += wbytes + 2.0 * hh * ww * 3.0 * 8.0;
    P.release(feat[l]);
    P.debug["aligned_side/" + std::to_string(l)] =
        DebugTensor{true, sd->hi, sd->lo, (int64_t)hh * ww, sd->C, 0, 10};
    for (int k = 0; k < 2; ++k)
      P.debug["warped" + std::to_string(k) + "/" + std::to_string(l)] =
          DebugTensor{true, o->hi + (int64_t)k * hh * ww * C, o->lo + (int64_t)k * hh * ww * C, (int64_t)hh * ww, C, 0, C};
  }
  auto batch_view = [&](const SplitBuf* b, int k) {
    P.bufs.emplace_back(new SplitBuf(*b));
    SplitBuf* s = P.bufs.back().get();
    s->B = 1;
    s->hi = b->hi + (int64_t)k * b->H * b->W * b->C;
    s->lo = b->lo + (int64_t)k * b->H * b->W * b->C;
    return (const SplitBuf*)s;
  };

  const SplitBuf* net = nullptr;
  for (int i = kFusionLevels - 2; i >= 0; --i) {
    const int nf = fusion_filters(i), hh = Hs[i], ww = Ws[i];
    const int cpad = round_up(nf, kChunk);
    SplitBuf* up = P.split(1, hh, ww, cpad);
    std::vector<SrcRef> up_src;
    if (i == kFusionLevels - 2)
      up_src = {{batch_view(wf[i + 1], 0), 0}, {batch_view(wf[i + 1], 1), 0}, {side[i + 1], 0}};
    else
      up_src = {{net, 0}};
    if (P.conv_impl == 0) {
      size_t first = 0;
      for (int py = 0; py < 2; ++py)
        for (int px = 0; px < 2; ++px) {
          const size_t ci = add_conv(P, "", 0, M.fus_up[i][py * 2 + px], up_src, 0, up, 0, ST_FUS + 3 * i, ST_FUS + 3 * i + 1, 2, 2,
                                     py, px, nullptr, true);
          if (py == 0 && px == 0) first = ci;
        }
      P.h_probs[first].group = 4;
      const double up_bytes = 4.0 * P.last_conv_bytes;
      Plan* pq = &P;
      const double fl = 2.0 * 16.0 * M.fus_up[i][0].cin_ref * nf * (double)Hs[i + 1] * Ws[i + 1];
      P.add_op(0, "fusion_up@L" + std::to_string(i), [pq, first](cudaStream_t st) {
        return launch_conv_tc(pq->d_probs + first, pq->h_probs[first], st);
      }, fl, up_bytes);
    } else {
      for (int py = 0; py < 2; ++py)
        for (int px = 0; px < 2; ++px)
          add_conv(P, "fusion_up" + std::to_string(py * 2 + px) + "@L" + std::to_string(i),
                   4.0 * M.fus_up[i][0].cin_ref * nf, M.fus_up[i][py * 2 + px], up_src, 0, up, 0, ST_FUS + 3 * i,
                   ST_FUS + 3 * i + 1, 2, 2, py, px);
    }
    const bool fuse_rgb = (i == 0) && P.conv_impl == 0 && P.conv3x3_v2 && P.fuse_rgb_head && !keep_debug;
    SplitBuf* f1 = P.split(1, hh, ww, cpad);
    SplitBuf* f2 = fuse_rgb ? nullptr : P.split(1, hh, ww, cpad);
    add_conv(P, "fusion_conv1@L" + std::to_string(i), 9.0 * M.fus_c1[i].cin_ref * nf, M.fus_c1[i],
             {{batch_view(wf[i], 0), 0}, {batch_view(wf[i], 1), 0}, {side[i], 0}, {up, 0}}, 1, f1, 0, ST_FUS + 3 * i + 1,
             ST_FUS + 3 * i + 2);
    if (fuse_rgb) {
      const size_t ci = add_conv(P, "fusion_conv2+rgb@L0", 9.0 * nf * nf + 64.0 * 3, M.fus_c2[i], {{f1, 0}}, 1, nullptr, 0,
                                 ST_FUS + 3 * i + 2, ST_NONE, 1, 1, 0, 0, nullptr, false, 2);
      ConvProblem& hp = P.h_probs[ci];
      if (hp.cout != 64 || hp.bn != 64) throw Error{FILM_ERR_UNSUPPORTED, "RGB-head epilogue expects a 64-channel N tile"};
      hp.head_w4 = M.rgb_w;
      hp.head_b4 = M.rgb_b;
      hp.head_v = P.xout;
      hp.crop_y = P.off_y;
      hp.crop_x = P.off_x;
      hp.crop_h = P.h;
      hp.crop_w = P.w;
      hp.crop_pitch = (int64_t)P.w * 3;
    } else {
      add_conv(P, "fusion_conv2@L" + std::to_string(i), 9.0 * nf * nf, M.fus_c2[i], {{f1, 0}}, 1, f2, 0, ST_FUS + 3 * i + 2,
               i > 0 ? ST_FUS + 3 * (i - 1) : ST_NONE);
    }
    if (i == kFusionLevels - 2) P.release(wf[i + 1]);
    else P.release(net);
    P.release(wf[i]);
    P.release(up);
    P.release(f1);
    net = f2;
    if (f2) P.debug["fusion_net/" + std::to_string(i)] = DebugTensor{true, f2->hi, f2->lo, (int64_t)hh * ww, f2->C, 0, nf};
    P.debug["fusion_up/" + std::to_string(i)] = DebugTensor{true, up->hi, up->lo, (int64_t)hh * ww, up->C, 0, nf};
  }
  {
    const float *rw = M.rgb_w, *rb = M.rgb_b;
    if (!(P.conv_impl == 0 && P.conv3x3_v2 && P.fuse_rgb_head && !keep_debug))
      P.add_op(2, "rgb_head", [=](cudaStream_t st) {
        return launch_rgb_head(net->hi, net->lo, net->C, pp->H, pp->W, rw, rb, pp->xout, (int64_t)pp->w * 3, pp->off_y,
                               pp->off_x, pp->h, pp->w, st);
      });
    P.debug["image"] = DebugTensor{false, P.xout, nullptr, (int64_t)h * w, 3, 0, 3};
    P.tok_end = P.new_token();
    P.signal_last(P.tok_end);
  }

  {
    double fe = 0, fl = 0, fu = 0;
    for (int i = 0; i < kLevels; ++i) {
      const int depth = (kLevels - i) < kSubLevels ? (kLevels - i) : kSubLevels;
      int cin = 3;
      for (int j = 0; j < depth; ++j) {
        const double c = kFilters << j;
        fe += (double)Hs[i + j] * Ws[i + j] * 9.0 * (cin * c + c * c);
        cin = (int)c;
      }
    }
    fe *= 2;
    for (int l = 0; l < kLevels; ++l) {
      const double nf = kFlowFilters[l < kSpecialized ? l : kSpecialized], cin = 2.0 * feat_channels(l);
      fl += (double)Hs[l] * Ws[l] * (9 * cin * nf + 18 * nf * nf + nf * nf / 2 + nf);
    }
    fl *= 2;
    for (int i = 0; i < kFusionLevels - 1; ++i) {
      const double nf = fusion_filters(i), a_c = 2.0 * (3 + feat_channels(i)) + 4;
      const double cc = (i == kFusionLevels - 2) ? 2.0 * (3 + feat_channels(i + 1)) + 4 : fusion_filters(i + 1);
      fu += (double)Hs[i] * Ws[i] * (4 * cc * nf + 9 * (a_c + nf) * nf + 9 * nf * nf);
    }
    fu += (double)Hs[0] * Ws[0] * 64 * 3;
    P.conv_flops = 2.0 * (fe + fl + fu);
  }

  if (P.reuse)
    for (auto& kv : P.debug)
      if (P.block_bytes.count((void*)kv.second.p0) ||
          kv.first.compare(0, 4, "feat") == 0 || kv.first.compare(0, 6, "warped") == 0 ||
          kv.first.compare(0, 11, "flow_warped") == 0 || kv.first.compare(0, 8, "flow_vup") == 0)
        kv.second.recycled = true;
  FILM_CUDA(cudaMalloc(&P.d_probs, P.h_probs.size() * sizeof(ConvProblem)));
  P.allocs.push_back(P.d_probs);
  FILM_CUDA(cudaMemcpy(P.d_probs, P.h_probs.data(), P.h_probs.size() * sizeof(ConvProblem), cudaMemcpyHostToDevice));
  (void)keep_debug;
  return pl;
}

}

using namespace film;

struct film_handle {
  int device = 0;
  cudaStream_t stream = nullptr;
  cudaEvent_t ev[4] = {nullptr, nullptr, nullptr, nullptr};
  std::unique_ptr<Model> model;
  std::map<std::string, std::unique_ptr<Plan>> plans;
  Plan* last_plan = nullptr;
  std::string err;
  int conv_impl = 0, use_graph = 1, keep_debug = 0, time_ops = 0;
  bool dev_events_valid = false;
  cudaStream_t copy_stream = nullptr;
  float* stage_in[2] = {nullptr, nullptr};
  float* stage_out[2] = {nullptr, nullptr};
  size_t stage_bytes = 0;
  cudaEvent_t ev_in[2] = {nullptr, nullptr}, ev_done[2] = {nullptr, nullptr}, ev_free[2] = {nullptr, nullptr},
              ev_out[2] = {nullptr, nullptr};
  cudaStream_t lane_streams[Plan::kNumLanes] = {};
  std::vector<cudaEvent_t> token_events;
  cudaEvent_t fork_event = nullptr;
  int use_lanes = 0;
  int conv3x3_v2 = 1;
  int conv3x3_2cta = 0;
  int conv3x3_halo = 3;
  uint32_t onepass_mask = kDefaultOnepassMask;
  int fe_conv0_tc = 0;
  int fuse_rgb_head = 1;
  int plane_skip = 1, mma_straight = 1, arena_reuse = 1;
  int fuse_flow_head = 1;
  uint8_t* u8_stage = nullptr;
  size_t u8_bytes = 0;
  int num_sms = 132;
  std::vector<cudaEvent_t> op_events;
  film_profile_t prof;
};

static std::string g_create_error;

static int fail(film_handle* h, const Error& e) noexcept {
  try {
    if (h) h->err = e.msg; else g_create_error = e.msg;
  } catch (...) {
  }
  return e.code;
}
#define FILM_CATCH_ALL(h)                                                                                     \
  catch (const Error& e) { return fail(h, e); }                                                               \
  catch (const std::bad_alloc&) { return fail(h, Error{FILM_ERR_CUDA, "out of host memory"}); }               \
  catch (const std::exception& e) { return fail(h, Error{FILM_ERR_CUDA, std::string("internal error: ") + e.what()}); } \
  catch (...) { return fail(h, Error{FILM_ERR_CUDA, "unknown internal error"}); }

static void enqueue_plan(film_handle* h, Plan* P, cudaStream_t origin) {
  if (!h->use_lanes) {
    for (auto& op : P->ops) FILM_CUDA(op.fn(origin));
    return;
  }
  if (!h->fork_event) FILM_CUDA(cudaEventCreateWithFlags(&h->fork_event, cudaEventDisableTiming));
  for (int i = 1; i < Plan::kNumLanes; ++i)
    if (!h->lane_streams[i]) FILM_CUDA(cudaStreamCreateWithFlags(&h->lane_streams[i], cudaStreamNonBlocking));
  while ((int)h->token_events.size() < P->num_tokens) {
    cudaEvent_t e;
    FILM_CUDA(cudaEventCreateWithFlags(&e, cudaEventDisableTiming));
    h->token_events.push_back(e);
  }
  auto lane_stream = [&](int lane) { return lane == 0 ? origin : h->lane_streams[lane]; };
  FILM_CUDA(cudaEventRecord(h->fork_event, origin));
  bool forked[Plan::kNumLanes] = {true};
  for (auto& op : P->ops) {
    cudaStream_t st = lane_stream(op.lane);
    if (!forked[op.lane]) {
      FILM_CUDA(cudaStreamWaitEvent(st, h->fork_event, 0));
      forked[op.lane] = true;
    }
    for (int t : op.waits) FILM_CUDA(cudaStreamWaitEvent(st, h->token_events[t], 0));
    FILM_CUDA(op.fn(st));
    for (int t : op.signals) FILM_CUDA(cudaEventRecord(h->token_events[t], st));
  }
  if (P->tok_end >= 0) FILM_CUDA(cudaStreamWaitEvent(origin, h->token_events[P->tok_end], 0));
}

static void drop_plans(film_handle* h) {
  cudaStreamSynchronize(h->stream);
  cudaDeviceSynchronize();
  (void)cudaGetLastError();
  h->last_plan = nullptr;
  h->dev_events_valid = false;
  h->plans.clear();
}

static Plan* get_plan(film_handle* h, int hh, int ww, int align) {
  char key[96];
  snprintf(key, sizeof(key), "%dx%d_a%d_i%d_v%d_l%d_p%d_h%d_m%x_d%d", hh, ww, align > 0 ? align : 0, h->conv_impl, h->conv3x3_v2,
           h->use_lanes, h->conv3x3_2cta, h->conv3x3_halo, h->onepass_mask, h->keep_debug * 256 + h->fuse_flow_head * 64 + h->arena_reuse * 32 + h->mma_straight * 16 + h->plane_skip * 8 +
               h->fuse_rgb_head * 2 + h->fe_conv0_tc);
  auto it = h->plans.find(key);
  if (it != h->plans.end()) return it->second.get();
  std::unique_ptr<Plan> p;
  try {
    p = build_plan(*h->model, hh, ww, align, h->conv_impl, h->keep_debug != 0, h->conv3x3_v2, h->num_sms,
                   h->conv3x3_2cta, h->conv3x3_halo, h->onepass_mask, h->use_lanes != 0, h->fe_conv0_tc | (h->fuse_rgb_head ? 0 : 2) | (h->plane_skip ? 0 : 8) |
                       (h->mma_straight ? 0 : 16) | (h->arena_reuse ? 0 : 32) | (h->fuse_flow_head ? 0 : 64) |
                       (h->fuse_flow_head >= 2 ? 128 : 0));
  } catch (const Error& e0) {
    if (e0.code != FILM_ERR_CUDA) throw;
    if (h->plans.empty()) throw;
    drop_plans(h);
    p = build_plan(*h->model, hh, ww, align, h->conv_impl, h->keep_debug != 0, h->conv3x3_v2, h->num_sms,
                   h->conv3x3_2cta, h->conv3x3_halo, h->onepass_mask, h->use_lanes != 0, h->fe_conv0_tc | (h->fuse_rgb_head ? 0 : 2) | (h->plane_skip ? 0 : 8) |
                       (h->mma_straight ? 0 : 16) | (h->arena_reuse ? 0 : 32) | (h->fuse_flow_head ? 0 : 64) |
                       (h->fuse_flow_head >= 2 ? 128 : 0));
  }
  if (h->use_graph) {
    cudaGraph_t g = nullptr;
    FILM_CUDA(cudaStreamBeginCapture(h->stream, cudaStreamCaptureModeThreadLocal));
    try {
      enqueue_plan(h, p.get(), h->stream);
    } catch (const Error& err) {
      cudaStreamEndCapture(h->stream, &g);
      if (g) cudaGraphDestroy(g);
      (void)cudaGetLastError();
      throw Error{FILM_ERR_CUDA, "kernel launch failed during capture: " + err.msg};
    }
    FILM_CUDA(cudaStreamEndCapture(h->stream, &g));
    FILM_CUDA(cudaGraphInstantiate(&p->graph, g, 0));
    cudaGraphDestroy(g);
  }
  Plan* raw = p.get();
  h->plans[key] = std::move(p);
  return raw;
}

static void run_plan(film_handle* h, Plan* P, cudaStream_t st) {
  if (P->graph && !h->time_ops) {
    FILM_CUDA(cudaGraphLaunch(P->graph, st));
  } else {
    if (h->time_ops && st == h->stream) {
      const size_t n = P->ops.size();
      while (h->op_events.size() < n + 1) {
        cudaEvent_t e;
        FILM_CUDA(cudaEventCreate(&e));
        h->op_events.push_back(e);
      }
      FILM_CUDA(cudaEventRecord(h->op_events[0], st));
      for (size_t i = 0; i < n; ++i) {
        FILM_CUDA(P->ops[i].fn(st));
        FILM_CUDA(cudaEventRecord(h->op_events[i + 1], st));
      }
      FILM_CUDA(cudaStreamSynchronize(st));
      P->op_ms.assign(n, 0.f);
      for (size_t i = 0; i < n; ++i) FILM_CUDA(cudaEventElapsedTime(&P->op_ms[i], h->op_events[i], h->op_events[i + 1]));
    } else {
      enqueue_plan(h, P, st);
    }
  }
  h->last_plan = P;
}

extern "C" {

const char* film_version(void) {
  return "film_b200 0.3 sm_90a split=" FILM_SPLIT_NAME
         " mma=wgmma.f32, per-stage precision plan: 3-pass (hi*hi+hi*lo+lo*hi) or 1-pass (hi*hi)";
}

int film_create(film_handle** out, const char* weights_path, int device_ordinal) {
  if (!out || !weights_path) {
    g_create_error = "null argument";
    return FILM_ERR_ARG;
  }
  *out = nullptr;
  film_handle* h = nullptr;
  try {
    int ndev = 0;
    if (cudaGetDeviceCount(&ndev) != cudaSuccess || ndev == 0)
      throw Error{FILM_ERR_CUDA, "no CUDA device: the FILM engine has no CPU fallback"};
    if (device_ordinal < 0 || device_ordinal >= ndev) throw Error{FILM_ERR_ARG, "bad device ordinal"};
    FILM_CUDA(cudaSetDevice(device_ordinal));
    cudaDeviceProp prop;
    FILM_CUDA(cudaGetDeviceProperties(&prop, device_ordinal));
    if (prop.major != 9 || prop.minor != 0)
      throw Error{FILM_ERR_CUDA, std::string("device is sm_") + std::to_string(prop.major * 10 + prop.minor) +
                                     ", this engine is sm_90a-only (wgmma/TMA)"};
    h = new film_handle;
    h->device = device_ordinal;
    memset(&h->prof, 0, sizeof(h->prof));
    FILM_CUDA(cudaStreamCreateWithFlags(&h->stream, cudaStreamNonBlocking));
    for (auto& e : h->ev) FILM_CUDA(cudaEventCreate(&e));
    FILM_CUDA(conv_tc_configure());
    FILM_CUDA(conv3x3_tc_configure());
    if (const char* e2 = getenv("FILM_2CTA")) h->conv3x3_2cta = atoi(e2);
    if (const char* e3 = getenv("FILM_HALO")) h->conv3x3_halo = atoi(e3);
    if (const char* e5 = getenv("FILM_FE0_TC")) h->fe_conv0_tc = atoi(e5) ? 1 : 0;
    if (const char* e6 = getenv("FILM_RGB_FUSE")) h->fuse_rgb_head = atoi(e6) ? 1 : 0;
    if (const char* e8 = getenv("FILM_PLANE_SKIP")) h->plane_skip = atoi(e8) ? 1 : 0;
    if (const char* e11 = getenv("FILM_FLOW_HEAD_FUSE")) h->fuse_flow_head = atoi(e11) < 0 ? 0 : (atoi(e11) > 2 ? 2 : atoi(e11));
    if (const char* e9 = getenv("FILM_STRAIGHT")) h->mma_straight = atoi(e9) ? 1 : 0;
    if (const char* e10 = getenv("FILM_ARENA_REUSE")) h->arena_reuse = atoi(e10) ? 1 : 0;
    if (const char* e4 = getenv("FILM_ONEPASS")) h->onepass_mask = (uint32_t)strtoul(e4, nullptr, 0);
    h->num_sms = prop.multiProcessorCount;
    WeightMap w = read_weight_file(weights_path);
    h->model.reset(new Model);
    h->model->load(w);
    *out = h;
    return FILM_OK;
  } catch (const Error& e) {
    fail(nullptr, e);
    if (h) film_destroy(h);
    return e.code;
  } catch (const std::exception& e) {
    fail(nullptr, Error{FILM_ERR_CUDA, std::string("internal error: ") + e.what()});
    if (h) film_destroy(h);
    return FILM_ERR_CUDA;
  } catch (...) {
    fail(nullptr, Error{FILM_ERR_CUDA, "unknown internal error"});
    if (h) film_destroy(h);
    return FILM_ERR_CUDA;
  }
}

void film_destroy(film_handle* h) {
  if (!h) return;
  cudaSetDevice(h->device);
  if (h->stream) cudaStreamSynchronize(h->stream);
  h->plans.clear();
  h->model.reset();
  for (auto& e : h->ev)
    if (e) cudaEventDestroy(e);
  for (auto& e : h->op_events) cudaEventDestroy(e);
  for (auto& e : h->token_events) cudaEventDestroy(e);
  for (int i = 0; i < 2; ++i) {
    if (h->stage_in[i]) cudaFree(h->stage_in[i]);
    if (h->stage_out[i]) cudaFree(h->stage_out[i]);
    for (cudaEvent_t e : {h->ev_in[i], h->ev_done[i], h->ev_free[i], h->ev_out[i]})
      if (e) cudaEventDestroy(e);
  }
  if (h->u8_stage) cudaFree(h->u8_stage);
  if (h->copy_stream) cudaStreamDestroy(h->copy_stream);
  if (h->fork_event) cudaEventDestroy(h->fork_event);
  for (int i = 1; i < Plan::kNumLanes; ++i)
    if (h->lane_streams[i]) cudaStreamDestroy(h->lane_streams[i]);
  if (h->stream) cudaStreamDestroy(h->stream);
  delete h;
}

const char* film_last_error(film_handle* h) { return h ? h->err.c_str() : g_create_error.c_str(); }

int film_set_option(film_handle* h, const char* name, int value) {
  if (!h || !name) return FILM_ERR_ARG;
  try {
  std::string n(name);
  if (n == "conv_impl") h->conv_impl = value;
  else if (n == "use_graph") h->use_graph = value;
  else if (n == "keep_debug") h->keep_debug = value;
  else if (n == "time_ops") h->time_ops = value;
  else if (n == "use_lanes") h->use_lanes = value;
  else if (n == "conv3x3_v2") h->conv3x3_v2 = value;
  else if (n == "conv3x3_2cta") h->conv3x3_2cta = value;
  else if (n == "conv3x3_halo") h->conv3x3_halo = value;
  else if (n == "onepass_mask") h->onepass_mask = (uint32_t)value & ((1u << ST_COUNT) - 1u);
  else if (n == "onepass_default") h->onepass_mask = kDefaultOnepassMask;
  else if (n == "fe_conv0_tc") h->fe_conv0_tc = value ? 1 : 0;
  else if (n == "fuse_rgb_head") h->fuse_rgb_head = value ? 1 : 0;
  else if (n == "plane_skip") h->plane_skip = value ? 1 : 0;
  else if (n == "fuse_flow_head") h->fuse_flow_head = value < 0 ? 0 : (value > 2 ? 2 : value);
  else if (n == "mma_straight") h->mma_straight = value ? 1 : 0;
  else if (n == "arena_reuse") h->arena_reuse = value ? 1 : 0;
  else if (n == "clear_plans") drop_plans(h);
  else {
    h->err = "unknown option " + n;
    return FILM_ERR_ARG;
  }
  return FILM_OK;
  }
  FILM_CATCH_ALL(h)
}

int film_stage_count(void) { return ST_COUNT; }

int film_stage_name(int stage, char* buf, int buf_size) {
  if (!buf || buf_size < 1 || stage < 0 || stage >= ST_COUNT) return FILM_ERR_ARG;
  try {
    const std::string n = stage_name(stage);
    snprintf(buf, (size_t)buf_size, "%s", n.c_str());
    return FILM_OK;
  } catch (...) {
    return FILM_ERR_CUDA;
  }
}

int film_get_option(film_handle* h, const char* name, int* value) {
  if (!h || !name || !value) return FILM_ERR_ARG;
  if (!strcmp(name, "onepass_mask")) *value = (int)h->onepass_mask;
  else if (!strcmp(name, "onepass_default")) *value = (int)kDefaultOnepassMask;
  else if (!strcmp(name, "conv3x3_halo")) *value = h->conv3x3_halo;
  else if (!strcmp(name, "conv3x3_2cta")) *value = h->conv3x3_2cta;
  else if (!strcmp(name, "keep_debug")) *value = h->keep_debug;
  else return FILM_ERR_ARG;
  return FILM_OK;
}

int film_synchronize(film_handle* h) {
  if (!h) return FILM_ERR_ARG;
  try {
    FILM_CUDA(cudaSetDevice(h->device));
    FILM_CUDA(cudaStreamSynchronize(h->stream));
    return FILM_OK;
  }
  FILM_CATCH_ALL(h)
}

extern "C++" {
static void ensure_staging(film_handle* h, size_t frame_bytes) {
  if (!h->copy_stream) FILM_CUDA(cudaStreamCreateWithFlags(&h->copy_stream, cudaStreamNonBlocking));
  for (int i = 0; i < 2; ++i) {
    if (!h->ev_in[i]) {
      FILM_CUDA(cudaEventCreateWithFlags(&h->ev_in[i], cudaEventDisableTiming));
      FILM_CUDA(cudaEventCreateWithFlags(&h->ev_done[i], cudaEventDisableTiming));
      FILM_CUDA(cudaEventCreateWithFlags(&h->ev_free[i], cudaEventDisableTiming));
      FILM_CUDA(cudaEventCreateWithFlags(&h->ev_out[i], cudaEventDisableTiming));
    }
  }
  if (h->stage_bytes >= frame_bytes) return;
  for (int i = 0; i < 2; ++i) {
    if (h->stage_in[i]) cudaFree(h->stage_in[i]);
    if (h->stage_out[i]) cudaFree(h->stage_out[i]);
    h->stage_in[i] = h->stage_out[i] = nullptr;
  }
  h->stage_bytes = 0;
  for (int i = 0; i < 2; ++i) {
    FILM_CUDA(cudaMalloc(&h->stage_in[i], 2 * frame_bytes));
    FILM_CUDA(cudaMalloc(&h->stage_out[i], frame_bytes));
  }
  h->stage_bytes = frame_bytes;
}

template <class Fetch, class Deliver>
static void run_pipelined(film_handle* h, Plan* P, int n, size_t frame_bytes, Fetch fetch, Deliver deliver) {
  ensure_staging(h, frame_bytes);
  cudaStream_t cs = h->copy_stream, ms = h->stream;
  FILM_CUDA(cudaStreamSynchronize(ms));
  FILM_CUDA(cudaStreamSynchronize(cs));
  for (int i = 0; i < n; ++i) {
    const int b = i & 1;
    if (i >= 2) FILM_CUDA(cudaStreamWaitEvent(cs, h->ev_free[b], 0));
    fetch(i, h->stage_in[b], (float*)((char*)h->stage_in[b] + frame_bytes), cs);
    FILM_CUDA(cudaEventRecord(h->ev_in[b], cs));
    FILM_CUDA(cudaStreamWaitEvent(ms, h->ev_in[b], 0));
    FILM_CUDA(cudaMemcpyAsync(P->xin, h->stage_in[b], 2 * frame_bytes, cudaMemcpyDeviceToDevice, ms));
    FILM_CUDA(cudaEventRecord(h->ev_free[b], ms));
    run_plan(h, P, ms);
    if (i >= 2) FILM_CUDA(cudaStreamWaitEvent(ms, h->ev_out[b], 0));
    FILM_CUDA(cudaMemcpyAsync(h->stage_out[b], P->xout, frame_bytes, cudaMemcpyDeviceToDevice, ms));
    FILM_CUDA(cudaEventRecord(h->ev_done[b], ms));
    if (i >= 1) {
      const int pb = (i - 1) & 1;
      FILM_CUDA(cudaStreamWaitEvent(cs, h->ev_done[pb], 0));
      deliver(i - 1, h->stage_out[pb], cs);
      FILM_CUDA(cudaEventRecord(h->ev_out[pb], cs));
    }
  }
  const int lb = (n - 1) & 1;
  FILM_CUDA(cudaStreamWaitEvent(cs, h->ev_done[lb], 0));
  deliver(n - 1, h->stage_out[lb], cs);
  FILM_CUDA(cudaStreamSynchronize(cs));
  FILM_CUDA(cudaStreamSynchronize(ms));
}

}

static void check_frame_args(const void* x0, const void* x1, const void* out, int B, int H, int W) {
  if (!x0 || !x1 || !out) throw Error{FILM_ERR_ARG, "null frame pointer"};
  if (B < 1 || H < 1 || W < 1) throw Error{FILM_ERR_ARG, "batch, height and width must be positive"};
}

static void fill_profile(film_handle* h, Plan* P, float ms_net, float ms_h2d, float ms_d2h) {
  film_profile_t& p = h->prof;
  p.last_call_ms = ms_net;
  p.last_h2d_ms = ms_h2d;
  p.last_d2h_ms = ms_d2h;
  p.conv_flops = P->conv_flops;
  p.mma_flops = P->mma_flops;
  p.warp_bytes = P->warp_bytes;
  p.kernel_launches = (int64_t)P->ops.size();
  p.arena_bytes = P->arena_bytes;
  p.padded_h = P->H;
  p.padded_w = P->W;
  p.used_graph = P->graph ? 1 : 0;
}

int film_interpolate(film_handle* h, const float* x0, const float* x1, const float* dt, int B, int H, int W,
                     int align, float* out) {
  if (!h) return FILM_ERR_ARG;
  (void)dt;
  try {
    check_frame_args(x0, x1, out, B, H, W);
    FILM_CUDA(cudaSetDevice(h->device));
    (void)cudaGetLastError();
    Plan* P = get_plan(h, H, W, align);
    const size_t frame = (size_t)H * W * 3 * sizeof(float);
    float ms_net = 0, ms_h2d = 0, ms_d2h = 0;
    if (B > 1 && !h->time_ops) {
      run_pipelined(h, P, B, frame,
                    [&](int b, float* d0, float* d1, cudaStream_t cs) {
                      FILM_CUDA(cudaMemcpyAsync(d0, (const char*)x0 + b * frame, frame, cudaMemcpyHostToDevice, cs));
                      FILM_CUDA(cudaMemcpyAsync(d1, (const char*)x1 + b * frame, frame, cudaMemcpyHostToDevice, cs));
                    },
                    [&](int b, const float* src, cudaStream_t cs) {
                      FILM_CUDA(cudaMemcpyAsync((char*)out + b * frame, src, frame, cudaMemcpyDeviceToHost, cs));
                    });
      fill_profile(h, P, 0.f, 0.f, 0.f);
      return FILM_OK;
    }
    for (int b = 0; b < B; ++b) {
      FILM_CUDA(cudaEventRecord(h->ev[0], h->stream));
      FILM_CUDA(cudaMemcpyAsync(P->xin, (const char*)x0 + b * frame, frame, cudaMemcpyHostToDevice, h->stream));
      FILM_CUDA(cudaMemcpyAsync((char*)P->xin + frame, (const char*)x1 + b * frame, frame, cudaMemcpyHostToDevice, h->stream));
      FILM_CUDA(cudaEventRecord(h->ev[1], h->stream));
      run_plan(h, P, h->stream);
      FILM_CUDA(cudaEventRecord(h->ev[2], h->stream));
      FILM_CUDA(cudaMemcpyAsync((char*)out + b * frame, P->xout, frame, cudaMemcpyDeviceToHost, h->stream));
      FILM_CUDA(cudaEventRecord(h->ev[3], h->stream));
      FILM_CUDA(cudaStreamSynchronize(h->stream));
      float t;
      FILM_CUDA(cudaEventElapsedTime(&t, h->ev[0], h->ev[1]));
      ms_h2d += t;
      FILM_CUDA(cudaEventElapsedTime(&t, h->ev[1], h->ev[2]));
      ms_net += t;
      FILM_CUDA(cudaEventElapsedTime(&t, h->ev[2], h->ev[3]));
      ms_d2h += t;
    }
    fill_profile(h, P, ms_net, ms_h2d, ms_d2h);
    return FILM_OK;
  }
  FILM_CATCH_ALL(h)
}

int film_interpolate_device(film_handle* h, const float* d_x0, const float* d_x1, int B, int H, int W,
                            int64_t in_pitch, int align, float* d_out, int64_t out_pitch, void* cuda_stream) {
  if (!h) return FILM_ERR_ARG;
  try {
    check_frame_args(d_x0, d_x1, d_out, B, H, W);
    if (in_pitch < (int64_t)W * 3 || out_pitch < (int64_t)W * 3) throw Error{FILM_ERR_ARG, "pitch smaller than a row"};
    FILM_CUDA(cudaSetDevice(h->device));
    (void)cudaGetLastError();
    Plan* P = get_plan(h, H, W, align);
    cudaStream_t st = cuda_stream ? (cudaStream_t)cuda_stream : h->stream;
    const size_t row = (size_t)W * 3 * sizeof(float);
    for (int b = 0; b < B; ++b) {
      FILM_CUDA(cudaMemcpy2DAsync(P->xin, row, d_x0 + (int64_t)b * H * in_pitch, in_pitch * 4, row, H,
                                  cudaMemcpyDeviceToDevice, st));
      FILM_CUDA(cudaMemcpy2DAsync(P->xin + (int64_t)H * W * 3, row, d_x1 + (int64_t)b * H * in_pitch, in_pitch * 4, row, H,
                                  cudaMemcpyDeviceToDevice, st));
      FILM_CUDA(cudaEventRecord(h->ev[1], st));
      run_plan(h, P, st);
      FILM_CUDA(cudaEventRecord(h->ev[2], st));
      FILM_CUDA(cudaMemcpy2DAsync(d_out + (int64_t)b * H * out_pitch, out_pitch * 4, P->xout, row, row, H,
                                  cudaMemcpyDeviceToDevice, st));
    }
    fill_profile(h, P, -1.f, 0.f, 0.f);
    h->dev_events_valid = true;
    return FILM_OK;
  }
  FILM_CATCH_ALL(h)
}

int film_interpolate_tiled(film_handle* h, const float* x0, const float* x1, const float* dt, int H, int W, int align,
                           int block_h, int block_w, float* out) {
  if (!h) return FILM_ERR_ARG;
  (void)dt;
  try {
    check_frame_args(x0, x1, out, 1, H, W);
    if (block_h < 1 || block_w < 1) throw Error{FILM_ERR_ARG, "block shape must be positive"};
    if (H % block_h) throw Error{FILM_ERR_ARG, "block_height=" + std::to_string(block_h) + " should evenly divide height=" + std::to_string(H) + "."};
    if (W % block_w) throw Error{FILM_ERR_ARG, "block_width=" + std::to_string(block_w) + " should evenly divide width=" + std::to_string(W) + "."};
    FILM_CUDA(cudaSetDevice(h->device));
    const int ph = H / block_h, pw = W / block_w;
    Plan* P = get_plan(h, ph, pw, align);
    const size_t row = (size_t)pw * 3 * sizeof(float), full_row = (size_t)W * 3 * sizeof(float);
    float ms_net = 0, ms_h2d = 0, ms_d2h = 0;
    if (block_h * block_w > 1 && !h->time_ops) {
      const size_t tile_bytes = (size_t)ph * pw * 3 * sizeof(float);
      auto tile_off = [&](int t) { return ((size_t)(t / block_w) * ph * W + (size_t)(t % block_w) * pw) * 3; };
      run_pipelined(h, P, block_h * block_w, tile_bytes,
                    [&](int t, float* d0, float* d1, cudaStream_t cs) {
                      FILM_CUDA(cudaMemcpy2DAsync(d0, row, x0 + tile_off(t), full_row, row, ph, cudaMemcpyHostToDevice, cs));
                      FILM_CUDA(cudaMemcpy2DAsync(d1, row, x1 + tile_off(t), full_row, row, ph, cudaMemcpyHostToDevice, cs));
                    },
                    [&](int t, const float* src, cudaStream_t cs) {
                      FILM_CUDA(cudaMemcpy2DAsync(out + tile_off(t), full_row, src, row, row, ph, cudaMemcpyDeviceToHost, cs));
                    });
      fill_profile(h, P, 0.f, 0.f, 0.f);
      return FILM_OK;
    }
    for (int r = 0; r < block_h; ++r)
      for (int c = 0; c < block_w; ++c) {
        const size_t off = ((size_t)r * ph * W + (size_t)c * pw) * 3;
        FILM_CUDA(cudaEventRecord(h->ev[0], h->stream));
        FILM_CUDA(cudaMemcpy2DAsync(P->xin, row, x0 + off, full_row, row, ph, cudaMemcpyHostToDevice, h->stream));
        FILM_CUDA(cudaMemcpy2DAsync(P->xin + (size_t)ph * pw * 3, row, x1 + off, full_row, row, ph, cudaMemcpyHostToDevice, h->stream));
        FILM_CUDA(cudaEventRecord(h->ev[1], h->stream));
        run_plan(h, P, h->stream);
        FILM_CUDA(cudaEventRecord(h->ev[2], h->stream));
        FILM_CUDA(cudaMemcpy2DAsync(out + off, full_row, P->xout, row, row, ph, cudaMemcpyDeviceToHost, h->stream));
        FILM_CUDA(cudaEventRecord(h->ev[3], h->stream));
        FILM_CUDA(cudaStreamSynchronize(h->stream));
        float t;
        FILM_CUDA(cudaEventElapsedTime(&t, h->ev[0], h->ev[1]));
        ms_h2d += t;
        FILM_CUDA(cudaEventElapsedTime(&t, h->ev[1], h->ev[2]));
        ms_net += t;
        FILM_CUDA(cudaEventElapsedTime(&t, h->ev[2], h->ev[3]));
        ms_d2h += t;
      }
    fill_profile(h, P, ms_net, ms_h2d, ms_d2h);
    return FILM_OK;
  }
  FILM_CATCH_ALL(h)
}

extern "C++" {
static int recursive_impl(film_handle* h, const void* frame0, const void* frame1, int H, int W, int align,
                          int times_to_interpolate, void* out, bool u8) {
  if (!h) return FILM_ERR_ARG;
  try {
    check_frame_args(frame0, frame1, out, 1, H, W);
    if (times_to_interpolate < 0 || times_to_interpolate > 10) throw Error{FILM_ERR_ARG, "times_to_interpolate must be in [0, 10]"};
    FILM_CUDA(cudaSetDevice(h->device));
    (void)cudaGetLastError();
    Plan* P = get_plan(h, H, W, align);
    const int n = (1 << times_to_interpolate) + 1;
    const int64_t elems = (int64_t)H * W * 3;
    const size_t frame = (size_t)elems * sizeof(float);
    const size_t io_frame = u8 ? (size_t)elems : frame;
    ensure_staging(h, 16);
    std::vector<std::pair<int, cudaEvent_t>> frame_events;
    float* seq = nullptr;
    uint8_t* q = nullptr;
    FILM_CUDA(cudaMalloc(&seq, frame * n));
    if (u8 && cudaMalloc(&q, io_frame * (n + 2)) != cudaSuccess) {
      cudaFree(seq);
      throw Error{FILM_ERR_CUDA, "out of device memory for the 8-bit frame staging"};
    }
    cudaError_t e = cudaSuccess;
    auto slot = [&](int i) { return (float*)((char*)seq + frame * i); };
    auto qslot = [&](int i) { return q + io_frame * (size_t)(i + 2); };
    auto chk = [&](cudaError_t x) { if (e == cudaSuccess) e = x; };
    chk(cudaEventRecord(h->ev[0], h->stream));
    if (u8) {
      chk(cudaMemcpyAsync(q, frame0, io_frame, cudaMemcpyHostToDevice, h->stream));
      chk(cudaMemcpyAsync(q + io_frame, frame1, io_frame, cudaMemcpyHostToDevice, h->stream));
      chk(launch_u8_to_f32(q, slot(0), elems, h->stream));
      chk(launch_u8_to_f32(q + io_frame, slot(n - 1), elems, h->stream));
    } else {
      chk(cudaMemcpyAsync(slot(0), frame0, frame, cudaMemcpyHostToDevice, h->stream));
      chk(cudaMemcpyAsync(slot(n - 1), frame1, frame, cudaMemcpyHostToDevice, h->stream));
    }
    chk(cudaEventRecord(h->ev[1], h->stream));
    for (int step = (n - 1) / 2; step >= 1 && e == cudaSuccess; step /= 2) {
      for (int i = step; i < n - 1 && e == cudaSuccess; i += 2 * step) {
        chk(cudaMemcpyAsync(P->xin, slot(i - step), frame, cudaMemcpyDeviceToDevice, h->stream));
        chk(cudaMemcpyAsync((char*)P->xin + frame, slot(i + step), frame, cudaMemcpyDeviceToDevice, h->stream));
        if (e == cudaSuccess) {
          try {
            run_plan(h, P, h->stream);
          } catch (...) {
            cudaStreamSynchronize(h->stream);
            for (auto& fe : frame_events) cudaEventDestroy(fe.second);
            cudaFree(seq);
            if (q) cudaFree(q);
            throw;
          }
        }
        chk(cudaMemcpyAsync(slot(i), P->xout, frame, cudaMemcpyDeviceToDevice, h->stream));
        if (u8) chk(launch_f32_to_u8(slot(i), qslot(i), elems, h->stream));
        if (e == cudaSuccess) {
          cudaEvent_t ev;
          chk(cudaEventCreateWithFlags(&ev, cudaEventDisableTiming));
          chk(cudaEventRecord(ev, h->stream));
          frame_events.push_back({i, ev});
        }
      }
    }
    chk(cudaEventRecord(h->ev[2], h->stream));
    memcpy(out, frame0, io_frame);
    memcpy((char*)out + io_frame * (n - 1), frame1, io_frame);
    for (auto& fe : frame_events) {
      chk(cudaStreamWaitEvent(h->copy_stream, fe.second, 0));
      chk(cudaMemcpyAsync((char*)out + io_frame * fe.first, u8 ? (const void*)qslot(fe.first) : (const void*)slot(fe.first),
                          io_frame, cudaMemcpyDeviceToHost, h->copy_stream));
    }
    chk(cudaStreamSynchronize(h->copy_stream));
    chk(cudaEventRecord(h->ev[3], h->stream));
    chk(cudaStreamSynchronize(h->stream));
    for (auto& fe : frame_events) cudaEventDestroy(fe.second);
    float t_h2d = 0, t_net = 0, t_d2h = 0;
    if (e == cudaSuccess) {
      cudaEventElapsedTime(&t_h2d, h->ev[0], h->ev[1]);
      cudaEventElapsedTime(&t_net, h->ev[1], h->ev[2]);
      cudaEventElapsedTime(&t_d2h, h->ev[2], h->ev[3]);
    }
    cudaFree(seq);
    if (q) cudaFree(q);
    FILM_CUDA(e);
    fill_profile(h, P, t_net, t_h2d, t_d2h);
    h->prof.kernel_launches = (int64_t)P->ops.size() * (n - 2);
    return FILM_OK;
  }
  FILM_CATCH_ALL(h)
}
}

int film_interpolate_recursive(film_handle* h, const float* frame0, const float* frame1, int H, int W, int align,
                               int times_to_interpolate, float* out) {
  return recursive_impl(h, frame0, frame1, H, W, align, times_to_interpolate, out, false);
}

int film_interpolate_recursive_u8(film_handle* h, const uint8_t* frame0, const uint8_t* frame1, int H, int W, int align,
                                  int times_to_interpolate, uint8_t* out) {
  return recursive_impl(h, frame0, frame1, H, W, align, times_to_interpolate, out, true);
}

int film_interpolate_u8(film_handle* h, const uint8_t* x0, const uint8_t* x1, int B, int H, int W, int align,
                        uint8_t* out) {
  if (!h) return FILM_ERR_ARG;
  try {
    check_frame_args(x0, x1, out, B, H, W);
    FILM_CUDA(cudaSetDevice(h->device));
    (void)cudaGetLastError();
    Plan* P = get_plan(h, H, W, align);
    const int64_t elems = (int64_t)H * W * 3;
    if (h->u8_bytes < (size_t)elems * 3) {
      if (h->u8_stage) cudaFree(h->u8_stage);
      h->u8_stage = nullptr;
      h->u8_bytes = 0;
      FILM_CUDA(cudaMalloc(&h->u8_stage, (size_t)elems * 3));
      h->u8_bytes = (size_t)elems * 3;
    }
    uint8_t* q = h->u8_stage;
    float ms_net = 0, ms_h2d = 0, ms_d2h = 0;
    for (int b = 0; b < B; ++b) {
      FILM_CUDA(cudaEventRecord(h->ev[0], h->stream));
      FILM_CUDA(cudaMemcpyAsync(q, x0 + (int64_t)b * elems, elems, cudaMemcpyHostToDevice, h->stream));
      FILM_CUDA(cudaMemcpyAsync(q + elems, x1 + (int64_t)b * elems, elems, cudaMemcpyHostToDevice, h->stream));
      FILM_CUDA(cudaEventRecord(h->ev[1], h->stream));
      FILM_CUDA(launch_u8_to_f32(q, P->xin, elems, h->stream));
      FILM_CUDA(launch_u8_to_f32(q + elems, P->xin + elems, elems, h->stream));
      run_plan(h, P, h->stream);
      FILM_CUDA(launch_f32_to_u8(P->xout, q + 2 * elems, elems, h->stream));
      FILM_CUDA(cudaEventRecord(h->ev[2], h->stream));
      FILM_CUDA(cudaMemcpyAsync(out + (int64_t)b * elems, q + 2 * elems, elems, cudaMemcpyDeviceToHost, h->stream));
      FILM_CUDA(cudaEventRecord(h->ev[3], h->stream));
      FILM_CUDA(cudaStreamSynchronize(h->stream));
      float t;
      FILM_CUDA(cudaEventElapsedTime(&t, h->ev[0], h->ev[1]));
      ms_h2d += t;
      FILM_CUDA(cudaEventElapsedTime(&t, h->ev[1], h->ev[2]));
      ms_net += t;
      FILM_CUDA(cudaEventElapsedTime(&t, h->ev[2], h->ev[3]));
      ms_d2h += t;
    }
    fill_profile(h, P, ms_net, ms_h2d, ms_d2h);
    return FILM_OK;
  }
  FILM_CATCH_ALL(h)
}

void* film_host_alloc(size_t bytes) {
  void* p = nullptr;
  if (cudaHostAlloc(&p, bytes ? bytes : 16, cudaHostAllocDefault) != cudaSuccess) {
    (void)cudaGetLastError();
    return nullptr;
  }
  return p;
}

void film_host_free(void* p) {
  if (p) cudaFreeHost(p);
}

int film_profile(film_handle* h, film_profile_t* out) {
  if (!h || !out) return FILM_ERR_ARG;
  if (h->prof.last_call_ms < 0 && h->last_plan && h->dev_events_valid) {
    float t = 0;
    if (cudaEventSynchronize(h->ev[2]) == cudaSuccess && cudaEventElapsedTime(&t, h->ev[1], h->ev[2]) == cudaSuccess)
      h->prof.last_call_ms = t;
    else
      (void)cudaGetLastError();
  }
  *out = h->prof;
  return FILM_OK;
}

int film_op_table(film_handle* h, char* buf, int64_t buf_size, int64_t* needed) {
  if (!h || !h->last_plan) return FILM_ERR_ARG;
  try {
  std::string out = "idx,category,name,ms,ref_flops,alg_bytes\n";
  Plan* P = h->last_plan;
  for (size_t i = 0; i < P->ops.size(); ++i) {
    char line[256];
    snprintf(line, sizeof(line), "%zu,%d,%s,%.6f,%.0f,%.0f\n", i, P->ops[i].category, P->ops[i].name.c_str(),
             i < P->op_ms.size() ? P->op_ms[i] : -1.f, P->ops[i].flops, P->ops[i].bytes);
    out += line;
  }
  if (needed) *needed = (int64_t)out.size() + 1;
  if (buf && buf_size > 0) {
    const size_t n = out.size() < (size_t)buf_size - 1 ? out.size() : (size_t)buf_size - 1;
    memcpy(buf, out.data(), n);
    buf[n] = 0;
  }
  return FILM_OK;
  }
  FILM_CATCH_ALL(h)
}

int film_debug_read(film_handle* h, const char* name, float* dst, int64_t* count) {
  if (!h || !name) return FILM_ERR_ARG;
  try {
    if (!h->last_plan) throw Error{FILM_ERR_ARG, "no call has been made yet"};
    auto it = h->last_plan->debug.find(name);
    if (it == h->last_plan->debug.end()) throw Error{FILM_ERR_ARG, std::string("unknown debug tensor ") + name};
    const DebugTensor& d = it->second;
    if (d.recycled)
      throw Error{FILM_ERR_ARG, std::string(name) + " lives in a recycled activation buffer: set option keep_debug = 1 "
                                                    "before the call to read intermediates"};
    const int64_t n = d.npix * d.Cn;
    if (count) *count = n;
    if (!dst) return FILM_OK;
    FILM_CUDA(cudaSetDevice(h->device));
    FILM_CUDA(cudaStreamSynchronize(h->stream));
    if (!d.split) {
      FILM_CUDA(cudaMemcpy(dst, d.p0, n * 4, cudaMemcpyDeviceToHost));
    } else {
      float* tmp;
      FILM_CUDA(cudaMalloc(&tmp, n * 4));
      cudaError_t e = launch_unsplit((const sp_t*)d.p0, (const sp_t*)d.p1, d.C, d.c_off, d.Cn, d.npix, tmp, h->stream);
      if (e == cudaSuccess) e = cudaStreamSynchronize(h->stream);
      if (e == cudaSuccess) e = cudaMemcpy(dst, tmp, n * 4, cudaMemcpyDeviceToHost);
      cudaFree(tmp);
      FILM_CUDA(e);
    }
    return FILM_OK;
  }
  FILM_CATCH_ALL(h)
}

}
```

frame_interpolation_b200/csrc/film_tc_ptx.cuh:

```cuda
#pragma once
#include <cuda.h>
#include <cuda_runtime.h>
#include <stdint.h>

#include "film_conv.h"

namespace film {
namespace tc {

__device__ __forceinline__ uint32_t smem_u32(const void* p) {
  return (uint32_t)__cvta_generic_to_shared(p);
}

__device__ __forceinline__ void mbar_init(uint32_t bar, uint32_t count) {
  asm volatile("mbarrier.init.shared::cta.b64 [%0], %1;" ::"r"(bar), "r"(count));
}
__device__ __forceinline__ void mbar_expect_tx(uint32_t bar, uint32_t bytes) {
  asm volatile("mbarrier.arrive.expect_tx.shared::cta.b64 _, [%0], %1;" ::"r"(bar), "r"(bytes)
               : "memory");
}
__device__ __forceinline__ bool mbar_try_wait(uint32_t bar, uint32_t parity) {
  uint32_t ok;
  asm volatile(
      "{\n\t.reg .pred p;\n\t"
      "mbarrier.try_wait.parity.shared::cta.b64 p, [%1], %2;\n\t"
      "selp.u32 %0, 1, 0, p;\n\t}"
      : "=r"(ok)
      : "r"(bar), "r"(parity)
      : "memory");
  return ok != 0;
}
__device__ __forceinline__ void mbar_wait(uint32_t bar, uint32_t parity) {
  if (mbar_try_wait(bar, parity)) return;
  const long long t0 = clock64();
  while (!mbar_try_wait(bar, parity)) {
    if (clock64() - t0 > 4000000000LL) __trap();
  }
}
__device__ __forceinline__ void mbar_arrive(uint32_t bar) {
  asm volatile("mbarrier.arrive.shared::cta.b64 _, [%0];" ::"r"(bar) : "memory");
}

__device__ __forceinline__ void tma_load_4d(uint32_t dst, const CUtensorMap* tm, uint32_t bar, int c0,
                                            int c1, int c2, int c3) {
  asm volatile(
      "cp.async.bulk.tensor.4d.shared::cluster.global.mbarrier::complete_tx::bytes"
      " [%0], [%1, {%3, %4, %5, %6}], [%2];"
      ::"r"(dst), "l"(tm), "r"(bar), "r"(c0), "r"(c1), "r"(c2), "r"(c3)
      : "memory");
}
__device__ __forceinline__ void tma_load_2d(uint32_t dst, const CUtensorMap* tm, uint32_t bar, int c0,
                                            int c1) {
  asm volatile(
      "cp.async.bulk.tensor.2d.shared::cluster.global.mbarrier::complete_tx::bytes"
      " [%0], [%1, {%3, %4}], [%2];"
      ::"r"(dst), "l"(tm), "r"(bar), "r"(c0), "r"(c1)
      : "memory");
}
__device__ __forceinline__ void tma_load_2d_mc(uint32_t dst, const CUtensorMap* tm, uint32_t bar, int c0, int c1,
                                               uint16_t mask) {
  asm volatile(
      "cp.async.bulk.tensor.2d.shared::cluster.global.mbarrier::complete_tx::bytes.multicast::cluster"
      " [%0], [%1, {%3, %4}], [%2], %5;"
      ::"r"(dst), "l"(tm), "r"(bar), "r"(c0), "r"(c1), "h"(mask)
      : "memory");
}
__device__ __forceinline__ uint32_t cluster_ctarank() {
  uint32_t r;
  asm volatile("mov.u32 %0, %%cluster_ctarank;" : "=r"(r));
  return r;
}
__device__ __forceinline__ void cluster_sync_all() {
  asm volatile("barrier.cluster.arrive.release.aligned;" ::: "memory");
  asm volatile("barrier.cluster.wait.acquire.aligned;" ::: "memory");
}
__device__ __forceinline__ uint32_t map_to_cta(uint32_t local_addr, uint32_t rank) {
  uint32_t r;
  asm volatile("mapa.shared::cluster.u32 %0, %1, %2;" : "=r"(r) : "r"(local_addr), "r"(rank));
  return r;
}
__device__ __forceinline__ void mbar_arrive_cluster(uint32_t cluster_addr) {
  asm volatile("mbarrier.arrive.release.cluster.shared::cluster.b64 _, [%0];" ::"r"(cluster_addr) : "memory");
}

__device__ __forceinline__ void tma_prefetch_4d(const CUtensorMap* tm, int c0, int c1, int c2, int c3) {
  asm volatile("cp.async.bulk.prefetch.tensor.4d.L2.global.tile [%0, {%1, %2, %3, %4}];" ::"l"(tm), "r"(c0),
               "r"(c1), "r"(c2), "r"(c3)
               : "memory");
}

template <int KC>
__device__ __forceinline__ uint64_t make_desc_sbo(uint32_t saddr, uint32_t sbo_bytes) {
  constexpr uint64_t kType = (KC == 64) ? 1 : 2;
  uint64_t d = 0;
  d |= (uint64_t)((saddr & 0x3FFFFu) >> 4);
  d |= (uint64_t)1 << 16;
  d |= (uint64_t)(sbo_bytes >> 4) << 32;
  d |= kType << 62;
  return d;
}
template <int KC>
__device__ __forceinline__ uint64_t make_desc_kc(uint32_t saddr) {
  return make_desc_sbo<KC>(saddr, KC == 64 ? 1024u : 512u);
}

struct RingPos {
  int stage = 0;
  uint32_t phase = 0;
  __device__ __forceinline__ void advance(int depth) {
    if (++stage == depth) {
      stage = 0;
      phase ^= 1u;
    }
  }
};

struct FastDiv {
  uint64_t mul;
  uint32_t d;
  bool fast;
  __device__ __forceinline__ FastDiv(int divisor, int max_x) : d((uint32_t)divisor) {
    fast = (uint64_t)(uint32_t)max_x * d < (1ull << 40);
    mul = ((1ull << 40) + d - 1) / d;
  }
  __device__ __forceinline__ void divmod(int x, int& q, int& r) const {
    const uint32_t qq = fast ? (uint32_t)(((uint64_t)(uint32_t)x * mul) >> 40) : (uint32_t)x / d;
    q = (int)qq;
    r = x - (int)(qq * d);
  }
};

__device__ __forceinline__ bool elect_one() {
  uint32_t pred;
  asm volatile(
      "{\n\t.reg .pred P;\n\t"
      "elect.sync _|P, 0xffffffff;\n\t"
      "selp.u32 %0, 1, 0, P;\n\t}"
      : "=r"(pred));
  return pred != 0;
}

#ifdef FILM_SPLIT_FP16
#define FILM_WGMMA_AB "f16.f16"
#else
#define FILM_WGMMA_AB "bf16.bf16"
#endif

__device__ __forceinline__ void wgmma_fence() { asm volatile("wgmma.fence.sync.aligned;" ::: "memory"); }
__device__ __forceinline__ void wgmma_commit() { asm volatile("wgmma.commit_group.sync.aligned;" ::: "memory"); }
template <int N>
__device__ __forceinline__ void wgmma_wait() {
  asm volatile("wgmma.wait_group.sync.aligned %0;" ::"n"(N) : "memory");
}
template <int R>
__device__ __forceinline__ void acc_fence(float* d) {
#pragma unroll
  for (int i = 0; i < R; ++i) asm volatile("" : "+f"(d[i])::"memory");
}

template <int N>
__device__ __forceinline__ void regs_dec() {
  asm volatile("setmaxnreg.dec.sync.aligned.u32 %0;" ::"n"(N));
}
template <int N>
__device__ __forceinline__ void regs_inc() {
  asm volatile("setmaxnreg.inc.sync.aligned.u32 %0;" ::"n"(N));
}

template <int N>
__device__ __forceinline__ void wgmma(float* d, uint64_t a, uint64_t b, uint32_t scale_d);
template <>
__device__ __forceinline__ void wgmma<32>(float* d, uint64_t a, uint64_t b, uint32_t scale_d) {
  asm volatile(
      "{\n\t.reg .pred p;\n\t"
      "setp.ne.b32 p, %18, 0;\n\t"
      "wgmma.mma_async.sync.aligned.m64n32k16.f32." FILM_WGMMA_AB " "
      "{%0, %1, %2, %3, %4, %5, %6, %7, %8, %9, %10, %11, %12, %13, %14, %15}, "
      "%16, %17, p, 1, 1, 0, 0;\n\t}"
      : "+f"(d[0]), "+f"(d[1]), "+f"(d[2]), "+f"(d[3]), "+f"(d[4]), "+f"(d[5]), "+f"(d[6]), "+f"(d[7]), "+f"(d[8]), "+f"(d[9]), "+f"(d[10]), "+f"(d[11]), "+f"(d[12]), "+f"(d[13]), "+f"(d[14]), "+f"(d[15])
      : "l"(a), "l"(b), "r"(scale_d));
}
template <>
__device__ __forceinline__ void wgmma<64>(float* d, uint64_t a, uint64_t b, uint32_t scale_d) {
  asm volatile(
      "{\n\t.reg .pred p;\n\t"
      "setp.ne.b32 p, %34, 0;\n\t"
      "wgmma.mma_async.sync.aligned.m64n64k16.f32." FILM_WGMMA_AB " "
      "{%0, %1, %2, %3, %4, %5, %6, %7, %8, %9, %10, %11, %12, %13, %14, %15, %16, %17, %18, %19, %20, %21, %22, %23, %24, %25, %26, %27, %28, %29, %30, %31}, "
      "%32, %33, p, 1, 1, 0, 0;\n\t}"
      : "+f"(d[0]), "+f"(d[1]), "+f"(d[2]), "+f"(d[3]), "+f"(d[4]), "+f"(d[5]), "+f"(d[6]), "+f"(d[7]), "+f"(d[8]), "+f"(d[9]), "+f"(d[10]), "+f"(d[11]), "+f"(d[12]), "+f"(d[13]), "+f"(d[14]), "+f"(d[15]), "+f"(d[16]), "+f"(d[17]), "+f"(d[18]), "+f"(d[19]), "+f"(d[20]), "+f"(d[21]), "+f"(d[22]), "+f"(d[23]), "+f"(d[24]), "+f"(d[25]), "+f"(d[26]), "+f"(d[27]), "+f"(d[28]), "+f"(d[29]), "+f"(d[30]), "+f"(d[31])
      : "l"(a), "l"(b), "r"(scale_d));
}
template <>
__device__ __forceinline__ void wgmma<128>(float* d, uint64_t a, uint64_t b, uint32_t scale_d) {
  asm volatile(
      "{\n\t.reg .pred p;\n\t"
      "setp.ne.b32 p, %66, 0;\n\t"
      "wgmma.mma_async.sync.aligned.m64n128k16.f32." FILM_WGMMA_AB " "
      "{%0, %1, %2, %3, %4, %5, %6, %7, %8, %9, %10, %11, %12, %13, %14, %15, %16, %17, %18, %19, %20, %21, %22, %23, %24, %25, %26, %27, %28, %29, %30, %31, %32, %33, %34, %35, %36, %37, %38, %39, %40, %41, %42, %43, %44, %45, %46, %47, %48, %49, %50, %51, %52, %53, %54, %55, %56, %57, %58, %59, %60, %61, %62, %63}, "
      "%64, %65, p, 1, 1, 0, 0;\n\t}"
      : "+f"(d[0]), "+f"(d[1]), "+f"(d[2]), "+f"(d[3]), "+f"(d[4]), "+f"(d[5]), "+f"(d[6]), "+f"(d[7]), "+f"(d[8]), "+f"(d[9]), "+f"(d[10]), "+f"(d[11]), "+f"(d[12]), "+f"(d[13]), "+f"(d[14]), "+f"(d[15]), "+f"(d[16]), "+f"(d[17]), "+f"(d[18]), "+f"(d[19]), "+f"(d[20]), "+f"(d[21]), "+f"(d[22]), "+f"(d[23]), "+f"(d[24]), "+f"(d[25]), "+f"(d[26]), "+f"(d[27]), "+f"(d[28]), "+f"(d[29]), "+f"(d[30]), "+f"(d[31]), "+f"(d[32]), "+f"(d[33]), "+f"(d[34]), "+f"(d[35]), "+f"(d[36]), "+f"(d[37]), "+f"(d[38]), "+f"(d[39]), "+f"(d[40]), "+f"(d[41]), "+f"(d[42]), "+f"(d[43]), "+f"(d[44]), "+f"(d[45]), "+f"(d[46]), "+f"(d[47]), "+f"(d[48]), "+f"(d[49]), "+f"(d[50]), "+f"(d[51]), "+f"(d[52]), "+f"(d[53]), "+f"(d[54]), "+f"(d[55]), "+f"(d[56]), "+f"(d[57]), "+f"(d[58]), "+f"(d[59]), "+f"(d[60]), "+f"(d[61]), "+f"(d[62]), "+f"(d[63])
      : "l"(a), "l"(b), "r"(scale_d));
}
template <>
__device__ __forceinline__ void wgmma<256>(float* d, uint64_t a, uint64_t b, uint32_t scale_d) {
  asm volatile(
      "{\n\t.reg .pred p;\n\t"
      "setp.ne.b32 p, %130, 0;\n\t"
      "wgmma.mma_async.sync.aligned.m64n256k16.f32." FILM_WGMMA_AB " "
      "{%0, %1, %2, %3, %4, %5, %6, %7, %8, %9, %10, %11, %12, %13, %14, %15, %16, %17, %18, %19, %20, %21, %22, %23, %24, %25, %26, %27, %28, %29, %30, %31, %32, %33, %34, %35, %36, %37, %38, %39, %40, %41, %42, %43, %44, %45, %46, %47, %48, %49, %50, %51, %52, %53, %54, %55, %56, %57, %58, %59, %60, %61, %62, %63, %64, %65, %66, %67, %68, %69, %70, %71, %72, %73, %74, %75, %76, %77, %78, %79, %80, %81, %82, %83, %84, %85, %86, %87, %88, %89, %90, %91, %92, %93, %94, %95, %96, %97, %98, %99, %100, %101, %102, %103, %104, %105, %106, %107, %108, %109, %110, %111, %112, %113, %114, %115, %116, %117, %118, %119, %120, %121, %122, %123, %124, %125, %126, %127}, "
      "%128, %129, p, 1, 1, 0, 0;\n\t}"
      : "+f"(d[0]), "+f"(d[1]), "+f"(d[2]), "+f"(d[3]), "+f"(d[4]), "+f"(d[5]), "+f"(d[6]), "+f"(d[7]), "+f"(d[8]), "+f"(d[9]), "+f"(d[10]), "+f"(d[11]), "+f"(d[12]), "+f"(d[13]), "+f"(d[14]), "+f"(d[15]), "+f"(d[16]), "+f"(d[17]), "+f"(d[18]), "+f"(d[19]), "+f"(d[20]), "+f"(d[21]), "+f"(d[22]), "+f"(d[23]), "+f"(d[24]), "+f"(d[25]), "+f"(d[26]), "+f"(d[27]), "+f"(d[28]), "+f"(d[29]), "+f"(d[30]), "+f"(d[31]), "+f"(d[32]), "+f"(d[33]), "+f"(d[34]), "+f"(d[35]), "+f"(d[36]), "+f"(d[37]), "+f"(d[38]), "+f"(d[39]), "+f"(d[40]), "+f"(d[41]), "+f"(d[42]), "+f"(d[43]), "+f"(d[44]), "+f"(d[45]), "+f"(d[46]), "+f"(d[47]), "+f"(d[48]), "+f"(d[49]), "+f"(d[50]), "+f"(d[51]), "+f"(d[52]), "+f"(d[53]), "+f"(d[54]), "+f"(d[55]), "+f"(d[56]), "+f"(d[57]), "+f"(d[58]), "+f"(d[59]), "+f"(d[60]), "+f"(d[61]), "+f"(d[62]), "+f"(d[63]), "+f"(d[64]), "+f"(d[65]), "+f"(d[66]), "+f"(d[67]), "+f"(d[68]), "+f"(d[69]), "+f"(d[70]), "+f"(d[71]), "+f"(d[72]), "+f"(d[73]), "+f"(d[74]), "+f"(d[75]), "+f"(d[76]), "+f"(d[77]), "+f"(d[78]), "+f"(d[79]), "+f"(d[80]), "+f"(d[81]), "+f"(d[82]), "+f"(d[83]), "+f"(d[84]), "+f"(d[85]), "+f"(d[86]), "+f"(d[87]), "+f"(d[88]), "+f"(d[89]), "+f"(d[90]), "+f"(d[91]), "+f"(d[92]), "+f"(d[93]), "+f"(d[94]), "+f"(d[95]), "+f"(d[96]), "+f"(d[97]), "+f"(d[98]), "+f"(d[99]), "+f"(d[100]), "+f"(d[101]), "+f"(d[102]), "+f"(d[103]), "+f"(d[104]), "+f"(d[105]), "+f"(d[106]), "+f"(d[107]), "+f"(d[108]), "+f"(d[109]), "+f"(d[110]), "+f"(d[111]), "+f"(d[112]), "+f"(d[113]), "+f"(d[114]), "+f"(d[115]), "+f"(d[116]), "+f"(d[117]), "+f"(d[118]), "+f"(d[119]), "+f"(d[120]), "+f"(d[121]), "+f"(d[122]), "+f"(d[123]), "+f"(d[124]), "+f"(d[125]), "+f"(d[126]), "+f"(d[127])
      : "l"(a), "l"(b), "r"(scale_d));
}

}
}
```

frame_interpolation_b200/interpolator.py:

```python
from __future__ import annotations

import ctypes as C
from typing import List, Optional

import numpy as np

from . import _lib, weights as _weights


def _fptr(a: np.ndarray):
    return a.ctypes.data_as(C.POINTER(C.c_float))


def image_to_patches(image: np.ndarray, block_shape: List[int]) -> np.ndarray:
    block_height, block_width = block_shape
    height, width, channel = image.shape[-3:]
    patch_height, patch_width = height // block_height, width // block_width
    assert height == (patch_height * block_height), \
        'block_height=%d should evenly divide height=%d.' % (block_height, height)
    assert width == (patch_width * block_width), \
        'block_width=%d should evenly divide width=%d.' % (block_width, width)
    x = np.reshape(image, (block_height, patch_height, block_width, patch_width, channel))
    x = np.transpose(x, (0, 2, 1, 3, 4))
    return np.ascontiguousarray(np.reshape(x, (block_height * block_width, patch_height, patch_width, channel)))


def patches_to_image(patches: np.ndarray, block_shape: List[int]) -> np.ndarray:
    block_height, block_width = block_shape
    patch_height, patch_width, channel = patches.shape[-3:]
    x = np.reshape(patches, (block_height, block_width, patch_height, patch_width, channel))
    x = np.transpose(x, (0, 2, 1, 3, 4))
    return np.ascontiguousarray(np.reshape(x, (1, block_height * patch_height, block_width * patch_width, channel)))


class _PinnedPool:

    def __init__(self, lib, keep: int = 4):
        self._lib = lib
        self._keep = keep
        self._idle = {}

    def _release(self, nbytes: int, ptr: int) -> None:
        idle = self._idle.setdefault(nbytes, [])
        if len(idle) < self._keep:
            idle.append(ptr)
        else:
            self._lib.film_host_free(C.c_void_p(ptr))

    def empty(self, shape) -> np.ndarray:
        import weakref
        n = int(np.prod(shape))
        nbytes = n * 4
        idle = self._idle.get(nbytes)
        ptr = idle.pop() if idle else self._lib.film_host_alloc(nbytes)
        if not ptr:
            return np.empty(shape, np.float32)
        buf = (C.c_float * n).from_address(ptr)
        arr = np.ctypeslib.as_array(buf).reshape(shape)
        weakref.finalize(buf, self._release, nbytes, ptr)
        return arr

    def close(self) -> None:
        for ptrs in self._idle.values():
            for ptr in ptrs:
                self._lib.film_host_free(C.c_void_p(ptr))
        self._idle = {}


class Interpolator:

    def __init__(self, model_path: str, align: Optional[int] = None,
                 block_shape: Optional[List[int]] = None, device: int = 0) -> None:
        self._lib = _lib.load()
        if model_path is None:
            raise ValueError("model_path is required: a FILMW1 weight file (tf_bundle.convert_saved_model), or the "
                             "explicit string 'synthetic[:seed]' for seeded random weights (tests / benchmarks only)")
        if str(model_path).startswith("synthetic"):
            seed = 1234
            if ":" in str(model_path):
                seed = int(str(model_path).split(":", 1)[1])
            model_path = _weights.ensure_synthetic_file(seed=seed)
        self._handle = C.c_void_p()
        st = self._lib.film_create(C.byref(self._handle), str(model_path).encode(), int(device))
        if st != 0:
            msg = self._lib.film_last_error(None).decode()
            self._handle = C.c_void_p()
            raise RuntimeError(f"film_create failed (status {st}): {msg}")
        self._align = align or None
        self._block_shape = block_shape or None
        self.device = int(device)
        self._pool = _PinnedPool(self._lib)

    def close(self) -> None:
        if getattr(self, "_handle", None) is not None and self._handle.value:
            self._lib.film_destroy(self._handle)
            self._handle = C.c_void_p()
            if getattr(self, "_pool", None) is not None:
                self._pool.close()

    def __del__(self):
        try:
            self.close()
        except Exception:
            pass

    def _check(self, st: int) -> None:
        if st == 0:
            return
        msg = self._lib.film_last_error(self._handle).decode()
        if st == 1:
            raise AssertionError(msg)
        raise RuntimeError(f"film engine error (status {st}): {msg}")

    @staticmethod
    def _prep(x0, x1, dt):
        assert np.ndim(x0) == 4 and np.ndim(x1) == 4, "expected (batch, height, width, channels)"
        x0 = np.ascontiguousarray(x0, dtype=np.float32)
        x1 = np.ascontiguousarray(x1, dtype=np.float32)
        assert x0.shape == x1.shape, "x0 and x1 must have the same shape"
        assert x0.shape[-1] == 3, "expected 3 colour channels"
        dt = np.ascontiguousarray(dt, dtype=np.float32).reshape(-1)
        assert dt.shape[0] == x0.shape[0], "dt must have one entry per batch element"
        return x0, x1, dt

    def interpolate(self, x0: np.ndarray, x1: np.ndarray, dt: np.ndarray) -> np.ndarray:
        if self._align is not None:
            assert self._align > 0, 'align must be a positive number.'
        x0, x1, dt = self._prep(x0, x1, dt)
        b, h, w, _ = x0.shape
        out = self._pool.empty(x0.shape)
        st = self._lib.film_interpolate(self._handle, _fptr(x0), _fptr(x1), _fptr(dt), b, h, w,
                                        int(self._align or 0), _fptr(out))
        self._check(st)
        return out

    def __call__(self, x0: np.ndarray, x1: np.ndarray, dt: np.ndarray) -> np.ndarray:
        if self._block_shape is not None and np.prod(self._block_shape) > 1:
            if self._align is not None:
                assert self._align > 0, 'align must be a positive number.'
            x0, x1, dt = self._prep(x0, x1, dt)
            assert x0.shape[0] == 1, "tiled interpolation expects batch size 1"
            _, h, w, _ = x0.shape
            bh, bw = int(self._block_shape[0]), int(self._block_shape[1])
            out = self._pool.empty(x0.shape)
            st = self._lib.film_interpolate_tiled(self._handle, _fptr(x0), _fptr(x1), _fptr(dt), h, w,
                                                  int(self._align or 0), bh, bw, _fptr(out))
            self._check(st)
            return out
        return self.interpolate(x0, x1, dt)

    def interpolate_device(self, d_x0: int, d_x1: int, batch: int, height: int, width: int,
                           d_out: int, in_pitch: Optional[int] = None,
                           out_pitch: Optional[int] = None, stream: int = 0) -> None:
        in_pitch = in_pitch or width * 3
        out_pitch = out_pitch or width * 3
        st = self._lib.film_interpolate_device(self._handle, C.c_void_p(d_x0), C.c_void_p(d_x1), batch,
                                               height, width, in_pitch, int(self._align or 0),
                                               C.c_void_p(d_out), out_pitch, C.c_void_p(stream))
        self._check(st)

    def interpolate_recursively(self, frame0: np.ndarray, frame1: np.ndarray,
                                times_to_interpolate: int) -> np.ndarray:
        if self._align is not None:
            assert self._align > 0, 'align must be a positive number.'
        assert self._block_shape is None or np.prod(self._block_shape) <= 1, \
            "device-resident recursion is the untiled path"
        f0 = np.ascontiguousarray(frame0, dtype=np.float32)
        f1 = np.ascontiguousarray(frame1, dtype=np.float32)
        assert f0.ndim == 3 and f0.shape == f1.shape and f0.shape[-1] == 3, "expected two (H, W, 3) frames"
        h, w, _ = f0.shape
        n = (1 << int(times_to_interpolate)) + 1
        out = self._pool.empty((n, h, w, 3))
        st = self._lib.film_interpolate_recursive(self._handle, _fptr(f0), _fptr(f1), h, w,
                                                  int(self._align or 0), int(times_to_interpolate), _fptr(out))
        self._check(st)
        return out

    def interpolate_u8(self, x0: np.ndarray, x1: np.ndarray) -> np.ndarray:
        if self._align is not None:
            assert self._align > 0, 'align must be a positive number.'
        assert np.ndim(x0) == 4 and np.ndim(x1) == 4, "expected (batch, height, width, channels)"
        x0 = np.ascontiguousarray(x0, dtype=np.uint8)
        x1 = np.ascontiguousarray(x1, dtype=np.uint8)
        assert x0.shape == x1.shape and x0.shape[-1] == 3
        b, h, w, _ = x0.shape
        out = np.empty(x0.shape, np.uint8)
        up = C.POINTER(C.c_uint8)
        st = self._lib.film_interpolate_u8(self._handle, x0.ctypes.data_as(up), x1.ctypes.data_as(up), b, h, w,
                                           int(self._align or 0), out.ctypes.data_as(up))
        self._check(st)
        return out

    def interpolate_recursively_u8(self, frame0: np.ndarray, frame1: np.ndarray, times_to_interpolate: int) -> np.ndarray:
        if self._align is not None:
            assert self._align > 0, 'align must be a positive number.'
        f0 = np.ascontiguousarray(frame0, dtype=np.uint8)
        f1 = np.ascontiguousarray(frame1, dtype=np.uint8)
        assert f0.ndim == 3 and f0.shape == f1.shape and f0.shape[-1] == 3, "expected two (H, W, 3) uint8 frames"
        h, w, _ = f0.shape
        n = (1 << int(times_to_interpolate)) + 1
        out = np.empty((n, h, w, 3), np.uint8)
        up = C.POINTER(C.c_uint8)
        st = self._lib.film_interpolate_recursive_u8(self._handle, f0.ctypes.data_as(up), f1.ctypes.data_as(up), h, w,
                                                     int(self._align or 0), int(times_to_interpolate), out.ctypes.data_as(up))
        self._check(st)
        return out

    def synchronize(self) -> None:
        self._check(self._lib.film_synchronize(self._handle))

    def set_option(self, name: str, value: int) -> None:
        self._check(self._lib.film_set_option(self._handle, name.encode(), int(value)))

    def get_option(self, name: str) -> int:
        v = C.c_int()
        self._check(self._lib.film_get_option(self._handle, name.encode(), C.byref(v)))
        return int(v.value)

    def stage_names(self) -> List[str]:
        out = []
        for i in range(self._lib.film_stage_count()):
            buf = C.create_string_buffer(32)
            self._lib.film_stage_name(i, buf, 32)
            out.append(buf.value.decode())
        return out

    def clear_cache(self) -> None:
        self.set_option("clear_plans", 1)

    def profile(self) -> dict:
        p = _lib.FilmProfile()
        self._check(self._lib.film_profile(self._handle, C.byref(p)))
        return {k: getattr(p, k) for k, _ in p._fields_ if k != "reserved"}

    def debug_read(self, name: str) -> np.ndarray:
        n = C.c_int64()
        self._check(self._lib.film_debug_read(self._handle, name.encode(), None, C.byref(n)))
        out = np.empty(n.value, np.float32)
        self._check(self._lib.film_debug_read(self._handle, name.encode(), _fptr(out), C.byref(n)))
        return out

    def op_table(self) -> List[dict]:
        n = C.c_int64()
        self._check(self._lib.film_op_table(self._handle, None, 0, C.byref(n)))
        buf = C.create_string_buffer(n.value)
        self._check(self._lib.film_op_table(self._handle, buf, n.value, C.byref(n)))
        rows = buf.value.decode().strip().split("\n")
        keys = rows[0].split(",")
        out = []
        for r in rows[1:]:
            v = r.split(",")
            out.append({"idx": int(v[0]), "category": int(v[1]), "name": v[2], "ms": float(v[3]),
                        "ref_flops": float(v[4]), "alg_bytes": float(v[5])})
        return out

    @property
    def version(self) -> str:
        return self._lib.film_version().decode()
```

Before: 19.26.

## Add pixels-on-N 3x3 conv variant for 64-output-channel layers

Adds a k_conv3x3_tc variant for Cout=64 convs that swaps the wgmma operands. Weights become the M=64 operand and pixels the N=128 operand, so each warpgroup covers 128 pixels over a 32x8 tile. A new epilogue transposes accumulators through shared memory with stmatrix.trans and writes 16-byte vectors, and handles the 2x2 pooling path with shuffles. The aim is better wgmma shape efficiency and less halo overhead per output pixel for the many 64-channel layers. The cost is an extra staging-smem region, more template instantiations, and exclusion from the 2-CTA pair mode.

```diff
diff --git a/frame_interpolation_b200/csrc/film_conv.h b/frame_interpolation_b200/csrc/film_conv.h
--- a/frame_interpolation_b200/csrc/film_conv.h
+++ b/frame_interpolation_b200/csrc/film_conv.h
@@ -70,6 +70,7 @@
   int passes;
   int straight;
   int out_lo_skip;
+  int pxn;
 };
 
 cudaError_t launch_conv_tc(const ConvProblem* d_prob, const ConvProblem& h_prob, cudaStream_t st);
diff --git a/frame_interpolation_b200/csrc/film_conv3x3_tc.cu b/frame_interpolation_b200/csrc/film_conv3x3_tc.cu
--- a/frame_interpolation_b200/csrc/film_conv3x3_tc.cu
+++ b/frame_interpolation_b200/csrc/film_conv3x3_tc.cu
@@ -15,11 +15,11 @@
 constexpr int kThreads = kConsumers + 128;
 __host__ __device__ constexpr int a_plane_bytes(int kc, int th, int tw) { return (th + 2) * tw * kc * 2; }
 __host__ __device__ constexpr int a_stage_bytes(int kc, int th, int tw) { return 2 * a_plane_bytes(kc, th, tw); }
-constexpr int kHaloW = 10, kHaloRows = 18;
-__host__ __device__ constexpr int halo_box_bytes(int kc) { return kHaloRows * kHaloW * kc * 2; }
-__host__ __device__ constexpr int halo_plane_bytes(int kc) { return (halo_box_bytes(kc) + 1023) & ~1023; }
+constexpr int kHaloW = 10;
+__host__ __device__ constexpr int halo_box_bytes(int kc, int th) { return (th + 2) * kHaloW * kc * 2; }
+__host__ __device__ constexpr int halo_plane_bytes(int kc, int th) { return (halo_box_bytes(kc, th) + 1023) & ~1023; }
 __host__ __device__ constexpr int a_stage_bytes_h(int kc, int th, int tw, int halo, int planes = 2) {
-  return planes * (halo ? halo_plane_bytes(kc) : a_plane_bytes(kc, th, tw));
+  return planes * (halo ? halo_plane_bytes(kc, th) : a_plane_bytes(kc, th, tw));
 }
 constexpr int kMaxRing = 8;
 constexpr int kSmemLimit = 227 * 1024;
@@ -27,24 +27,30 @@
 constexpr int kFixedBytes = kBarBytes + 16 + 512 * 4  + 64  + 1024  + 64;
 constexpr int kHeadW3 = 64 * 32 * 4, kHeadMisc = 512;
 constexpr int kHeadBytes = kHeadW3 + kHeadMisc;
+constexpr int kPxnStageWg = 64 * 64 * 2;
+constexpr int kPxnStageBytes = 2 * kPxnStageWg;
+inline int epi_scratch_bytes(int epi_mode, int pxn) { return epi_mode == 3 ? kHeadBytes : pxn ? kPxnStageBytes : 0; }
 
 __host__ __device__ inline int w_tap_bytes(int bn, int kc, int planes = 2) { return bn * kc * 2 * planes; }
 
-template <int BN, int KC, bool kPartial, bool kHalo, bool kOne, bool kRes>
+template <int BN, int KC, bool kPartial, bool kHalo, bool kOne, bool kRes, bool kPxN = false>
 __global__ void __launch_bounds__(kThreads, 1) k_conv3x3_tc(const ConvProblem* __restrict__ prob) {
+  static_assert(!kPxN || (BN == 64 && KC == 64), "pixels on N: Cout = 64 (one M = 64 weight tile), 64-channel chunks");
   extern __shared__ uint8_t smem_raw[];
   constexpr bool one = kOne;
   const int planes = one ? 1 : 2;
   constexpr int kWPlane = BN * KC * 2;
   const int kWTap = kWPlane * planes;
   const int kTileH = prob->tile_h, kTileW = prob->tile_w;
-  constexpr int kHaloBox = halo_box_bytes(KC), kHaloPlane = halo_plane_bytes(KC);
+  constexpr int kHaloTileH = kPxN ? 32 : 16;
+  constexpr int kHaloBox = halo_box_bytes(KC, kHaloTileH), kHaloPlane = halo_plane_bytes(KC, kHaloTileH);
   constexpr bool halo = kHalo;
   const int kAPlane = halo ? kHaloPlane : a_plane_bytes(KC, kTileH, kTileW);
   const int kAStage = planes * kAPlane;
   const int kRowStep = kTileW * KC * 2;
-  constexpr bool kFused = BN <= 128;
-  constexpr int kAccRegs = (kFused ? 2 * BN : BN) / 2;
+  constexpr bool kFused = BN <= 128 && !kPxN;
+  constexpr int kAccRegs = kPxN ? 64 : (kFused ? 2 * BN : BN) / 2;
+  constexpr int kWgPx = kPxN ? 128 : 64;
 
   const int NA = prob->v2_na, NW = prob->v2_nw;
   const bool resident = prob->v2_resident != 0;
@@ -242,7 +248,7 @@
     constexpr uint32_t kPx = KC * 2;
     const int nab = nkb / kStageTaps;
     [[maybe_unused]] const int part_lo = prob->v2_part_lo, part_hi = prob->v2_part_hi;
-    const uint32_t a_row0 = kHalo ? (uint32_t)(wg * 8 * kHaloW) * kPx : (uint32_t)(wg * 64) * kPx;
+    const uint32_t a_row0 = kHalo ? (uint32_t)(wg * (kWgPx / 8) * kHaloW) * kPx : (uint32_t)(wg * kWgPx) * kPx;
     const uint32_t sbo = kHalo ? kHaloW * kPx : 8 * kPx;
     RingPos ra, rw;
     float acc[kAccRegs];
@@ -281,7 +287,13 @@
             for (int k = 0; k < kSteps; ++k) {
               const uint64_t adv = (uint64_t)(k * 32 >> 4);
               const uint32_t accf = (t == 0 && k == 0) ? first : 1u;
-              if constexpr (kOne) {
+              if constexpr (kPxN) {
+                wgmma<128>(acc, w_hi + adv, a_hi + adv, accf);
+                if constexpr (!kOne) {
+                  wgmma<128>(acc, w_lo + adv, a_hi + adv, 1u);
+                  wgmma<128>(acc, w_hi + adv, a_lo + adv, 1u);
+                }
+              } else if constexpr (kOne) {
                 wgmma<BN>(acc, a_hi + adv, w_hi + adv, accf);
               } else if constexpr (kFused) {
                 wgmma<BN>(acc, a_hi + adv, w_hi + adv, accf);
@@ -316,7 +328,13 @@
 #pragma unroll
             for (int k = 0; k < kSteps; ++k) {
               const uint64_t adv = (uint64_t)(k * 32 >> 4);
-              if constexpr (kOne) {
+              if constexpr (kPxN) {
+                wgmma<128>(acc, w_hi + adv, a_hi + adv, k == 0 ? first : 1u);
+                if constexpr (!kOne) {
+                  wgmma<128>(acc, w_lo + adv, a_hi + adv, 1u);
+                  wgmma<128>(acc, w_hi + adv, a_lo + adv, 1u);
+                }
+              } else if constexpr (kOne) {
                 wgmma<BN>(acc, a_hi + adv, w_hi + adv, k == 0 ? first : 1u);
               } else if constexpr (kFused) {
                 wgmma<BN>(acc, a_hi + adv, w_hi + adv, k == 0 ? first : 1u);
@@ -355,6 +373,76 @@
       div_tx.divmod(rem, ty, tx);
       const int n0 = nti * BN;
       const bool live = sp < nsp;
+      if constexpr (kPxN) {
+        const int c0 = 16 * (warp & 3) + (lane >> 2);
+        const float bias0 = bias_smem[c0], bias1 = bias_smem[c0 + 8];
+#pragma unroll
+        for (int i = 0; i < kAccRegs; ++i) {
+          const float f = acc[i] + ((i & 2) ? bias1 : bias0);
+          acc[i] = act ? leaky(f) : f;
+        }
+        const int y_wg = ty * kTileH + 16 * wg, x_t = tx * kTileW;
+        if (do_pool) {
+          const int px = x_t + 2 * q;
+#pragma unroll
+          for (int j = 0; j < 16; j += 2) {
+            const int py = y_wg + j;
+            const bool ok = live && py < H && px < W && !(lane & 4);
+            const int64_t ppix = ((int64_t)b * (out_H >> 1) + (py >> 1)) * (out_W >> 1) + (px >> 1);
+#pragma unroll
+            for (int h = 0; h < 2; ++h) {
+              const int i = 4 * j + 2 * h;
+              const float v = ((acc[i] + acc[i + 1]) + (acc[i + 4] + acc[i + 5])) * 0.25f;
+              const float vn = __shfl_xor_sync(0xffffffffu, v, 4);
+              if (ok) {
+                uint32_t hi, lo;
+                split_pack2(v, vn, hi, lo);
+                *reinterpret_cast<uint32_t*>(pool_hi + ppix * pool_C + c0 + 8 * h) = hi;
+                *reinterpret_cast<uint32_t*>(pool_lo + ppix * pool_C + c0 + 8 * h) = lo;
+              }
+            }
+          }
+        }
+        uint8_t* const stg = reinterpret_cast<uint8_t*>(src_tab) + 64 + wg * kPxnStageWg;
+        const uint32_t stg_u = smem_u32(stg);
+        const int t128 = threadIdx.x & 127;
+        auto wg_sync = [&]() { asm volatile("bar.sync %0, 128;" ::"r"(2 + wg) : "memory"); };
+        for (int pl = 0; pl < (lo_skip ? 1 : 2); ++pl) {
+          sp_t* const dst = pl ? out_lo : out_hi;
+#pragma unroll
+          for (int half = 0; half < 2; ++half) {
+            wg_sync();
+#pragma unroll
+            for (int jj = 0; jj < 8; jj += 2) {
+              uint32_t r[4];
+#pragma unroll
+              for (int m = 0; m < 4; ++m) {
+                const int i = 4 * (8 * half + jj + (m >> 1)) + 2 * (m & 1);
+                if (pl) {
+                  uint32_t hi;
+                  split_pack2(acc[i], acc[i + 1], hi, r[m]);
+                } else {
+                  r[m] = pack2_hi(acc[i], acc[i + 1]);
+                }
+              }
+              const int p = 8 * (jj + (lane >> 4)) + (lane & 7), ch = 2 * (warp & 3) + ((lane >> 3) & 1);
+              stmatrix_x4_trans(stg_u + p * 128 + ((ch ^ (p & 7)) << 4), r[0], r[1], r[2], r[3]);
+            }
+            wg_sync();
+#pragma unroll
+            for (int k = 0; k < 4; ++k) {
+              const int idx = 128 * k + t128, p = idx >> 3, ch = idx & 7;
+              const int py = y_wg + 8 * half + (p >> 3), px = x_t + (p & 7);
+              if (live && py < H && px < W) {
+                const uint4 v = *reinterpret_cast<const uint4*>(stg + p * 128 + ((ch ^ (p & 7)) << 4));
+                const int64_t opix = ((int64_t)b * out_H + py) * out_W + px;
+                *reinterpret_cast<uint4*>(dst + opix * out_C + out_c_off + 8 * ch) = v;
+              }
+            }
+          }
+        }
+        continue;
+      }
       auto value = [&](int h, int j, int e) {
         const int i = 4 * j + 2 * h + e;
         return (kFused && !kOne) ? acc[i] + acc[(i + BN / 2) % kAccRegs] : acc[i];
@@ -498,7 +586,7 @@
   const int planes = h.passes == 1 ? 1 : 2;
   const int w = h.v2_resident ? nkb * w_tap_bytes(bn, h.kchunk, planes) : h.v2_nw * w_tap_bytes(bn, h.kchunk, planes);
   return h.v2_na * a_stage_bytes_h(h.kchunk, h.tile_h, h.tile_w, h.halo, planes) + w + kFixedBytes +
-         (h.epi_mode == 3 ? kHeadBytes : 0);
+         epi_scratch_bytes(h.epi_mode, h.pxn);
 }
 
 }
@@ -506,11 +594,11 @@
 int conv_tc_block_n(int cout);
 
 namespace {
-bool ring_depths(int kc, int tile_h, int tile_w, int halo, int planes, int bn, int cout, int ktot, int epi_mode,
+bool ring_depths(int kc, int tile_h, int tile_w, int halo, int planes, int bn, int cout, int ktot, int epi_mode, int pxn,
                  int& resident, int& na, int& nw) {
   const int wtap = w_tap_bytes(bn, kc, planes);
   const int w_all = (ktot / kc) * wtap;
-  const int kLimit = kSmemLimit - (epi_mode == 3 ? kHeadBytes : 0);
+  const int kLimit = kSmemLimit - epi_scratch_bytes(epi_mode, pxn);
   const int kAStage = a_stage_bytes_h(kc, tile_h, tile_w, halo, planes);
   if (cout <= bn && w_all + 2 * kAStage + kFixedBytes <= kLimit) {
     resident = 1;
@@ -542,7 +630,7 @@
   tile_w = 8;
   for (auto& c : cand) {
     int res, na, nw;
-    if (!ring_depths(kc, c[0], c[1], 0, passes == 1 ? 1 : 2, bn, cout, ktot, epi_mode, res, na, nw)) continue;
+    if (!ring_depths(kc, c[0], c[1], 0, passes == 1 ? 1 : 2, bn, cout, ktot, epi_mode, 0, res, na, nw)) continue;
     const long tiles = (long)B * ((H + c[0] - 1) / c[0]) * ((W + c[1] - 1) / c[1]) * n_nt;
     const long waves = (tiles + num_sms - 1) / num_sms;
     const double cost = (double)waves * (c[0] + 2.0) / c[0] * (1.0 + 1e-3 * (c[1] / 8));
@@ -560,17 +648,17 @@
   const int wtap = w_tap_bytes(bn, h.kchunk, planes);
   const int w_all = (h.ktot / h.kchunk) * wtap;
   const bool can_resident = h.cout <= bn;
-  const int kLimit = kSmemLimit - (h.epi_mode == 3 ? kHeadBytes : 0);
-  if (h.halo && (h.tile_h != 16 || h.tile_w != 8 ||
+  const int kLimit = kSmemLimit - epi_scratch_bytes(h.epi_mode, h.pxn);
+  if (h.halo && (h.tile_h != (h.pxn ? 32 : 16) || h.tile_w != 8 ||
                  (can_resident && w_all + 2 * a_stage_bytes_h(h.kchunk, h.tile_h, h.tile_w, 0, planes) + kFixedBytes <= kLimit &&
                   w_all + 2 * a_stage_bytes_h(h.kchunk, h.tile_h, h.tile_w, 1, planes) + kFixedBytes > kLimit)))
     h.halo = 0;
-  bool ok = ring_depths(h.kchunk, h.tile_h, h.tile_w, h.halo, planes, bn, h.cout, h.ktot, h.epi_mode, h.v2_resident,
-                        h.v2_na, h.v2_nw);
+  bool ok = ring_depths(h.kchunk, h.tile_h, h.tile_w, h.halo, planes, bn, h.cout, h.ktot, h.epi_mode, h.pxn,
+                        h.v2_resident, h.v2_na, h.v2_nw);
   if (!ok && h.halo) {
     h.halo = 0;
-    ok = ring_depths(h.kchunk, h.tile_h, h.tile_w, 0, planes, bn, h.cout, h.ktot, h.epi_mode, h.v2_resident, h.v2_na,
-                     h.v2_nw);
+    ok = ring_depths(h.kchunk, h.tile_h, h.tile_w, 0, planes, bn, h.cout, h.ktot, h.epi_mode, h.pxn, h.v2_resident,
+                     h.v2_na, h.v2_nw);
   }
   const int nsp = h.B * h.tiles_y * h.tiles_x, n_nt = (h.cout + bn - 1) / bn;
   if (h.pair) {
@@ -582,17 +670,17 @@
   return ok;
 }
 
-template <int BN, int KC>
+template <int BN, int KC, bool kPxN = false>
 struct Variants {
   static constexpr void (*kFn[16])(const ConvProblem*) = {
-      k_conv3x3_tc<BN, KC, false, false, false, false>, k_conv3x3_tc<BN, KC, false, false, false, true>,
-      k_conv3x3_tc<BN, KC, false, false, true, false>,  k_conv3x3_tc<BN, KC, false, false, true, true>,
-      k_conv3x3_tc<BN, KC, false, true, false, false>,  k_conv3x3_tc<BN, KC, false, true, false, true>,
-      k_conv3x3_tc<BN, KC, false, true, true, false>,   k_conv3x3_tc<BN, KC, false, true, true, true>,
-      k_conv3x3_tc<BN, KC, true, false, false, false>,  k_conv3x3_tc<BN, KC, true, false, false, true>,
-      k_conv3x3_tc<BN, KC, true, false, true, false>,   k_conv3x3_tc<BN, KC, true, false, true, true>,
-      k_conv3x3_tc<BN, KC, true, true, false, false>,   k_conv3x3_tc<BN, KC, true, true, false, true>,
-      k_conv3x3_tc<BN, KC, true, true, true, false>,    k_conv3x3_tc<BN, KC, true, true, true, true>};
+      k_conv3x3_tc<BN, KC, false, false, false, false, kPxN>, k_conv3x3_tc<BN, KC, false, false, false, true, kPxN>,
+      k_conv3x3_tc<BN, KC, false, false, true, false, kPxN>,  k_conv3x3_tc<BN, KC, false, false, true, true, kPxN>,
+      k_conv3x3_tc<BN, KC, false, true, false, false, kPxN>,  k_conv3x3_tc<BN, KC, false, true, false, true, kPxN>,
+      k_conv3x3_tc<BN, KC, false, true, true, false, kPxN>,   k_conv3x3_tc<BN, KC, false, true, true, true, kPxN>,
+      k_conv3x3_tc<BN, KC, true, false, false, false, kPxN>,  k_conv3x3_tc<BN, KC, true, false, false, true, kPxN>,
+      k_conv3x3_tc<BN, KC, true, false, true, false, kPxN>,   k_conv3x3_tc<BN, KC, true, false, true, true, kPxN>,
+      k_conv3x3_tc<BN, KC, true, true, false, false, kPxN>,   k_conv3x3_tc<BN, KC, true, true, false, true, kPxN>,
+      k_conv3x3_tc<BN, KC, true, true, true, false, kPxN>,    k_conv3x3_tc<BN, KC, true, true, true, true, kPxN>};
   static cudaError_t configure() {
     for (auto fn : kFn) {
       const cudaError_t e = cudaFuncSetAttribute(fn, cudaFuncAttributeMaxDynamicSharedMemorySize, kSmemLimit);
@@ -602,6 +690,7 @@
   }
   static cudaError_t launch(const ConvProblem* d_prob, const ConvProblem& h, cudaStream_t st) {
     if (h.v2_na < 2 || (!h.v2_resident && h.v2_nw < 2)) return cudaErrorInvalidValue;
+    if (kPxN && (h.pair || h.tile_h != 32 || h.tile_w != 8 || h.epi_mode != 0)) return cudaErrorInvalidValue;
     const bool partial = h.v2_part_hi > h.v2_part_lo;
     const int idx = (partial ? 8 : 0) | (h.halo ? 4 : 0) | (h.passes == 1 ? 2 : 0) | (h.v2_resident && h.straight ? 1 : 0);
     if (!h.pair) {
@@ -631,6 +720,8 @@
   if (e != cudaSuccess) return e;
   FILM_CFG(32, 64) FILM_CFG(64, 64) FILM_CFG(128, 64) FILM_CFG(256, 64) FILM_CFG(32, 32) FILM_CFG(64, 32)
 #undef FILM_CFG
+  e = Variants<64, 64, true>::configure();
+  if (e != cudaSuccess) return e;
   return cudaSuccess;
 }
 
@@ -644,7 +735,7 @@
   switch (bn) {
     case 256: return Variants<256, 64>::launch(d_prob, h, st);
     case 128: return Variants<128, 64>::launch(d_prob, h, st);
-    case 64: return Variants<64, 64>::launch(d_prob, h, st);
+    case 64: return h.pxn ? Variants<64, 64, true>::launch(d_prob, h, st) : Variants<64, 64>::launch(d_prob, h, st);
     default: return Variants<32, 64>::launch(d_prob, h, st);
   }
 }
diff --git a/frame_interpolation_b200/csrc/film_engine.cu b/frame_interpolation_b200/csrc/film_engine.cu
--- a/frame_interpolation_b200/csrc/film_engine.cu
+++ b/frame_interpolation_b200/csrc/film_engine.cu
@@ -423,6 +423,7 @@
   int fuse_flow_head = 1;
   int plane_skip = 1;
   int mma_straight = 1;
+  int conv3x3_pxn = 1;
   std::vector<void*> allocs;
   int64_t arena_bytes = 0;
   std::vector<ConvProblem> h_probs;
@@ -436,6 +437,7 @@
     int lane;
     std::vector<int> waits;
     std::vector<int> signals;
+    std::string form = "";
   };
   std::vector<Op> ops;
   std::vector<float> op_ms;
@@ -539,9 +541,19 @@
   const bool v2 = P.conv3x3_v2 && P.conv_impl == 0 && pc.ntaps == 9 && (out || epi_mode >= 2) && sy == 1 && sx == 1 &&
                   (kc == kChunk || pc.cout <= 64);
   cp.epi_mode = epi_mode;
+  const long pxn_tiles = (long)cp.B * ((cp.H + 31) / 32) * ((cp.W + 7) / 8);
+  bool skips_ksteps = false;
+  for (size_t s = 0; s < pc.src_chunks.size(); ++s)
+    if (pc.src_chunks[s] > 0 && pc.src_ksteps[s] != kc / 16) skips_ksteps = true;
+  cp.pxn = (v2 && P.conv3x3_pxn && pc.cout == 64 && kc == kChunk && epi_mode == 0 && out && out_c_off % 8 == 0 &&
+            out->C % 8 == 0 && (!pool_out || pool_out->C % 8 == 0) &&
+            (P.conv3x3_pxn >= 2 || (pxn_tiles >= 2L * P.num_sms && !skips_ksteps))) ? 1 : 0;
   int box_h, box_w;
   if (v2) {
-    if (pool_out) {
+    if (cp.pxn) {
+      cp.tile_h = 32;
+      cp.tile_w = 8;
+    } else if (pool_out) {
       cp.tile_h = 16;
       cp.tile_w = 8;
     } else {
@@ -614,12 +626,12 @@
     cp.pool_C = pool_out->C;
   }
   cp.group = 1;
-  int halo_ok = (v2 && cp.tile_h == 16 && cp.tile_w == 8) ? P.conv3x3_halo : 0;
+  int halo_ok = (v2 && cp.tile_h == (cp.pxn ? 32 : 16) && cp.tile_w == 8) ? P.conv3x3_halo : 0;
   if (kc != kChunk && halo_ok < 3) halo_ok = 0;
   cp.halo = halo_ok >= 2;
   if (v2 && !conv3x3_tc_plan(cp, P.num_sms))
     throw Error{FILM_ERR_UNSUPPORTED, "persistent 3x3 conv: shared-memory rings do not fit (" + tag + ")"};
-  if (v2 && P.conv3x3_2cta && epi_mode < 2 && !cp.v2_resident &&
+  if (v2 && P.conv3x3_2cta && epi_mode < 2 && !cp.v2_resident && !cp.pxn &&
       (P.conv3x3_2cta >= 2 || (long)cp.B * cp.tiles_y * cp.tiles_x >= 4L * P.num_sms)) {
     cp.pair = 1;
     if (halo_ok >= 1) cp.halo = 1;
@@ -649,7 +661,7 @@
   double k_issued = 0;
   for (size_t si = 0; si < pc.src_chunks.size(); ++si)
     k_issued += (double)pc.src_chunks[si] * pc.ntaps * (v2 ? pc.src_ksteps[si] * 16 : pc.kchunk);
-  P.mma_flops += (double)cp.passes * 2.0 * (double)cp.B * cp.tiles_y * cp.tiles_x * kTileM * k_issued *
+  P.mma_flops += (double)cp.passes * 2.0 * (double)cp.B * cp.tiles_y * cp.tiles_x * (cp.tile_h * cp.tile_w) * k_issued *
                  (double)(((pc.cout + bn - 1) / bn) * bn);
   double alg_bytes = 0;
   {
@@ -670,6 +682,7 @@
     return v2 ? launch_conv3x3_tc(pp->d_probs + idx, pp->h_probs[idx], st)
               : launch_conv_tc(pp->d_probs + idx, pp->h_probs[idx], st);
   }, 2.0 * ref_macs_per_px * (double)cp.B * cp.H * cp.W, alg_bytes);
+  P.ops.back().form = impl == 1 ? "simt" : !v2 ? "tc" : cp.pxn ? "3x3_pxn" : "3x3";
   return idx;
 }
 
@@ -683,6 +696,7 @@
   P.plane_skip = (fe_conv0_tc & 8) ? 0 : 1;
   P.fuse_flow_head = (fe_conv0_tc & 64) ? 0 : ((fe_conv0_tc & 128) ? 2 : 1);
   P.mma_straight = (fe_conv0_tc & 16) ? 0 : 1;
+  P.conv3x3_pxn = (fe_conv0_tc >> 8) & 3;
   P.onepass_mask = onepass_mask;
   P.reuse = !keep_debug && !use_lanes && !(fe_conv0_tc & 32);
   P.h = h;
@@ -1096,6 +1110,7 @@
   int fuse_rgb_head = 1;
   int plane_skip = 1, mma_straight = 1, arena_reuse = 1;
   int fuse_flow_head = 1;
+  int conv3x3_pxn = 1;
   uint8_t* u8_stage = nullptr;
   size_t u8_bytes = 0;
   int num_sms = 132;
@@ -1159,7 +1174,7 @@
 static Plan* get_plan(film_handle* h, int hh, int ww, int align) {
   char key[96];
   snprintf(key, sizeof(key), "%dx%d_a%d_i%d_v%d_l%d_p%d_h%d_m%x_d%d", hh, ww, align > 0 ? align : 0, h->conv_impl, h->conv3x3_v2,
-           h->use_lanes, h->conv3x3_2cta, h->conv3x3_halo, h->onepass_mask, h->keep_debug * 256 + h->fuse_flow_head * 64 + h->arena_reuse * 32 + h->mma_straight * 16 + h->plane_skip * 8 +
+           h->use_lanes, h->conv3x3_2cta, h->conv3x3_halo, h->onepass_mask, h->conv3x3_pxn * 512 + h->keep_debug * 256 + h->fuse_flow_head * 64 + h->arena_reuse * 32 + h->mma_straight * 16 + h->plane_skip * 8 +
                h->fuse_rgb_head * 2 + h->fe_conv0_tc);
   auto it = h->plans.find(key);
   if (it != h->plans.end()) return it->second.get();
@@ -1168,7 +1183,7 @@
     p = build_plan(*h->model, hh, ww, align, h->conv_impl, h->keep_debug != 0, h->conv3x3_v2, h->num_sms,
                    h->conv3x3_2cta, h->conv3x3_halo, h->onepass_mask, h->use_lanes != 0, h->fe_conv0_tc | (h->fuse_rgb_head ? 0 : 2) | (h->plane_skip ? 0 : 8) |
                        (h->mma_straight ? 0 : 16) | (h->arena_reuse ? 0 : 32) | (h->fuse_flow_head ? 0 : 64) |
-                       (h->fuse_flow_head >= 2 ? 128 : 0));
+                       (h->fuse_flow_head >= 2 ? 128 : 0) | (h->conv3x3_pxn << 8));
   } catch (const Error& e0) {
     if (e0.code != FILM_ERR_CUDA) throw;
     if (h->plans.empty()) throw;
@@ -1176,7 +1191,7 @@
     p = build_plan(*h->model, hh, ww, align, h->conv_impl, h->keep_debug != 0, h->conv3x3_v2, h->num_sms,
                    h->conv3x3_2cta, h->conv3x3_halo, h->onepass_mask, h->use_lanes != 0, h->fe_conv0_tc | (h->fuse_rgb_head ? 0 : 2) | (h->plane_skip ? 0 : 8) |
                        (h->mma_straight ? 0 : 16) | (h->arena_reuse ? 0 : 32) | (h->fuse_flow_head ? 0 : 64) |
-                       (h->fuse_flow_head >= 2 ? 128 : 0));
+                       (h->fuse_flow_head >= 2 ? 128 : 0) | (h->conv3x3_pxn << 8));
   }
   if (h->use_graph) {
     cudaGraph_t g = nullptr;
@@ -1332,6 +1347,7 @@
   else if (n == "plane_skip") h->plane_skip = value ? 1 : 0;
   else if (n == "fuse_flow_head") h->fuse_flow_head = value < 0 ? 0 : (value > 2 ? 2 : value);
   else if (n == "mma_straight") h->mma_straight = value ? 1 : 0;
+  else if (n == "conv3x3_pxn") h->conv3x3_pxn = value < 0 ? 0 : (value > 2 ? 2 : value);
   else if (n == "arena_reuse") h->arena_reuse = value ? 1 : 0;
   else if (n == "clear_plans") drop_plans(h);
   else {
@@ -1362,6 +1378,7 @@
   else if (!strcmp(name, "onepass_default")) *value = (int)kDefaultOnepassMask;
   else if (!strcmp(name, "conv3x3_halo")) *value = h->conv3x3_halo;
   else if (!strcmp(name, "conv3x3_2cta")) *value = h->conv3x3_2cta;
+  else if (!strcmp(name, "conv3x3_pxn")) *value = h->conv3x3_pxn;
   else if (!strcmp(name, "keep_debug")) *value = h->keep_debug;
   else return FILM_ERR_ARG;
   return FILM_OK;
@@ -1762,12 +1779,12 @@
 int film_op_table(film_handle* h, char* buf, int64_t buf_size, int64_t* needed) {
   if (!h || !h->last_plan) return FILM_ERR_ARG;
   try {
-  std::string out = "idx,category,name,ms,ref_flops,alg_bytes\n";
+  std::string out = "idx,category,name,ms,ref_flops,alg_bytes,form\n";
   Plan* P = h->last_plan;
   for (size_t i = 0; i < P->ops.size(); ++i) {
     char line[256];
-    snprintf(line, sizeof(line), "%zu,%d,%s,%.6f,%.0f,%.0f\n", i, P->ops[i].category, P->ops[i].name.c_str(),
-             i < P->op_ms.size() ? P->op_ms[i] : -1.f, P->ops[i].flops, P->ops[i].bytes);
+    snprintf(line, sizeof(line), "%zu,%d,%s,%.6f,%.0f,%.0f,%s\n", i, P->ops[i].category, P->ops[i].name.c_str(),
+             i < P->op_ms.size() ? P->op_ms[i] : -1.f, P->ops[i].flops, P->ops[i].bytes, P->ops[i].form.c_str());
     out += line;
   }
   if (needed) *needed = (int64_t)out.size() + 1;
diff --git a/frame_interpolation_b200/csrc/film_tc_ptx.cuh b/frame_interpolation_b200/csrc/film_tc_ptx.cuh
--- a/frame_interpolation_b200/csrc/film_tc_ptx.cuh
+++ b/frame_interpolation_b200/csrc/film_tc_ptx.cuh
@@ -158,6 +158,12 @@
   for (int i = 0; i < R; ++i) asm volatile("" : "+f"(d[i])::"memory");
 }
 
+__device__ __forceinline__ void stmatrix_x4_trans(uint32_t addr, uint32_t r0, uint32_t r1, uint32_t r2, uint32_t r3) {
+  asm volatile("stmatrix.sync.aligned.m8n8.x4.trans.shared.b16 [%0], {%1, %2, %3, %4};" ::"r"(addr), "r"(r0), "r"(r1),
+               "r"(r2), "r"(r3)
+               : "memory");
+}
+
 template <int N>
 __device__ __forceinline__ void regs_dec() {
   asm volatile("setmaxnreg.dec.sync.aligned.u32 %0;" ::"n"(N));
diff --git a/frame_interpolation_b200/interpolator.py b/frame_interpolation_b200/interpolator.py
--- a/frame_interpolation_b200/interpolator.py
+++ b/frame_interpolation_b200/interpolator.py
@@ -251,7 +251,7 @@
         for r in rows[1:]:
             v = r.split(",")
             out.append({"idx": int(v[0]), "category": int(v[1]), "name": v[2], "ms": float(v[3]),
-                        "ref_flops": float(v[4]), "alg_bytes": float(v[5])})
+                        "ref_flops": float(v[4]), "alg_bytes": float(v[5]), "form": v[6]})
         return out
 
     @property
```

Result: faster. 19.90, median of 6 (+3.3%).
